# cloneofsimo/paint-with-words-sd

Hardware: AMD Instinct MI355X
Metric: 512x512 images/sec (30 steps, CFG) SD1.5+PwW (higher is better)
Workload: dtype bf16

## Files before the change

### paint-with-words-sd_amd/build.py

```python
import os
import subprocess
import sys

HERE = os.path.dirname(os.path.abspath(__file__))
REPO = os.path.dirname(HERE)
CSRC = os.path.join(HERE, "csrc")
LIB = os.path.join(HERE, "pww_hip", "libpww_hip.so")
LIB_EXPERIMENTS = os.path.join(HERE, "pww_hip", "libpww_hip_experiments.so")
UNITS = [("pww_api.hip", [], ""), ("pww_attn.hip", [], ""), ("pww_cross.hip", [], ""), ("pww_cross_lean.hip", [], ""), ("pww_reduce.hip", [], ""),
         ("pww_mask.hip", [], ""), ("pww_qproj.hip", [], ""), ("pww_norm.hip", [], ""), ("pww_blocks.hip", [], ""), ("pww_conv.hip", [], ""), ("pww_probs.hip", [], ""),
         ("pww_attn_inst.hip", ["-DPWW_INST_F16"], ".f16"), ("pww_attn_inst.hip", ["-DPWW_INST_BF16"], ".bf16"),
         ("pww_cross_inst.hip", ["-DPWW_INST_F16", "-DPWW_INST_NW=2"], ".f16.nw2"), ("pww_cross_inst.hip", ["-DPWW_INST_F16", "-DPWW_INST_NW=4"], ".f16.nw4"),
         ("pww_cross_inst.hip", ["-DPWW_INST_BF16", "-DPWW_INST_NW=2"], ".bf16.nw2"), ("pww_cross_inst.hip", ["-DPWW_INST_BF16", "-DPWW_INST_NW=4"], ".bf16.nw4")]
EXPERIMENT_UNITS = [("pww_cross_out.hip", [], "")]
_ATTN_HEADERS = ["pww_tile.h", "pww_attn_core.h", "pww_cross_tile.h"]
SIDE_FLAGS = ["-fvisibility=hidden"]
SIDE_LIBS = {
    "long": ("pww_long.hip", _ATTN_HEADERS, "the long-prompt launches"),
    "scope": ("pww_scope.hip", _ATTN_HEADERS, "cross-attention with per-head / per-row score statistics"),
    "linear": ("pww_linear.hip", [], "linear layers with a bias / residual / GEGLU epilogue"),
    "regions": ("pww_regions.hip", [], "region masks and the per-pixel blend of the noise predictions"),
    "lora": ("pww_lora.hip", [], "the per-row low-rank update of unmerged LoRA adapters"),
}
SIDE_LIBS_CONV = {
    "convtail": ("pww_conv_tail.hip", [], "conv2 of a ResnetBlock2D with the 1 x 1 shortcut as further K-slabs"),
}
SIDE_LIBS_EXTRA = {
    "canvas": ("pww_canvas.hip", [], "canvases larger than the UNet's window: the windows' gather and the combine of their noise predictions"),
}
ALL_SIDE_LIBS = {**SIDE_LIBS, **SIDE_LIBS_CONV, **SIDE_LIBS_EXTRA}
SOURCES = sorted({u[0] for u in UNITS + EXPERIMENT_UNITS})
HEADERS = ["pww_common.h", "pww_tile.h", "pww_attn_core.h", "pww_attn_kernel.h", "pww_cross_tile.h", "pww_cross_kernel.h", os.path.join(REPO, "include", "pww_hip.h")]
SIDE_PATHS = {n: os.path.join(HERE, "pww_hip", "libpww_hip_%s.so" % n) for n in ALL_SIDE_LIBS}
SIDE_UNITS = {n: [(v[0], SIDE_FLAGS, "")] for n, v in ALL_SIDE_LIBS.items()}
LIB_LONG, LIB_SCOPE, LIB_LINEAR, LIB_REGIONS, LIB_LORA = (SIDE_PATHS[n] for n in ("long", "scope", "linear", "regions", "lora"))
LONG_UNITS, SCOPE_UNITS, LINEAR_UNITS, REGIONS_UNITS, LORA_UNITS = (SIDE_UNITS[n] for n in ("long", "scope", "linear", "regions", "lora"))
LIB_CONVTAIL, CONVTAIL_UNITS = SIDE_PATHS["convtail"], SIDE_UNITS["convtail"]
LIB_CANVAS, CANVAS_UNITS = SIDE_PATHS["canvas"], SIDE_UNITS["canvas"]
SIDE_PUBLIC_HEADERS = {"canvas": ["pww_hip_regions.h"]}
HIPCC = os.environ.get("HIPCC", "/opt/rocm/bin/hipcc")
FLAGS = ["--offload-arch=gfx950", "-O3", "-std=c++17", "-fPIC", "-Wall",
         "-Wno-unused-function", "-mllvm", "-amdgpu-kernarg-preload-count=16"]


PER_FILE_FLAGS = {"pww_mask.hip": ["-ffp-contract=off"], "pww_regions.hip": ["-ffp-contract=off"], "pww_canvas.hip": ["-ffp-contract=off"]}


def _newer(target, deps):
    if not os.path.exists(target):
        return True
    t = os.path.getmtime(target)
    return any(os.path.getmtime(d) > t for d in deps)


def _deps():
    return ([os.path.join(CSRC, s) for s in SOURCES] + [h if os.path.isabs(h) else os.path.join(CSRC, h) for h in HEADERS] + [__file__])


def _build(lib, units, defines, objdir, verbose, jobs=None):
    os.makedirs(objdir, exist_ok=True)
    order = sorted(units, key=lambda u: {"pww_cross_inst.hip": 0, "pww_attn_inst.hip": 1, "pww_cross_lean.hip": 2}.get(u[0], 3))
    jobs = jobs or max(2, min(len(order), os.cpu_count() or 4, int(os.environ.get("MAX_JOBS", 16))))
    pending, running, objs = list(order), [], []
    while pending or running:
        while pending and len(running) < jobs:
            src, defs, suffix = pending.pop(0)
            o = os.path.join(objdir, src + suffix + ".o")
            objs.append(o)
            cmd = [HIPCC] + FLAGS + defines + defs + PER_FILE_FLAGS.get(src, []) + ["-c", os.path.join(CSRC, src), "-o", o]
            if verbose:
                print(" ".join(cmd))
            running.append((cmd, subprocess.Popen(cmd, stdout=subprocess.PIPE, stderr=subprocess.STDOUT, text=True)))
        cmd, p = running.pop(0)
        out, _ = p.communicate()
        if p.returncode != 0:
            for _, q in running:
                q.kill()
            raise RuntimeError("hipcc failed: %s\n%s" % (" ".join(cmd), out))
        if verbose and out.strip():
            print(out)
    subprocess.run([HIPCC, "--offload-arch=gfx950", "-shared", "-fPIC", "-s"] + sorted(objs) + ["-o", lib], check=True)
    return lib


def build_lib(force=False, verbose=False):
    if not force and not _newer(LIB, _deps()):
        return LIB
    return _build(LIB, UNITS, [], os.path.join(HERE, "build"), verbose)


def build_experiments(force=False, verbose=False):
    if not force and not _newer(LIB_EXPERIMENTS, _deps()):
        return LIB_EXPERIMENTS
    return _build(LIB_EXPERIMENTS, UNITS + EXPERIMENT_UNITS, ["-DPWW_EXPERIMENTS=1"], os.path.join(HERE, "build", "experiments"), verbose)


def build_side(name, force=False, verbose=False):
    unit, headers, _ = ALL_SIDE_LIBS[name]
    lib = SIDE_PATHS[name]
    public = ["pww_hip.h", "pww_hip_%s.h" % name] + SIDE_PUBLIC_HEADERS.get(name, [])
    deps = [os.path.join(CSRC, f) for f in [unit, "pww_common.h", "pww_side_host.h"] + headers] + [os.path.join(REPO, "include", h) for h in public] + [__file__]
    if not force and not _newer(lib, deps):
        return lib
    return _build(lib, SIDE_UNITS[name], [], os.path.join(HERE, "build", name), verbose)


def build_long(force=False, verbose=False): return build_side("long", force, verbose)
def build_scope(force=False, verbose=False): return build_side("scope", force, verbose)
def build_linear(force=False, verbose=False): return build_side("linear", force, verbose)
def build_regions(force=False, verbose=False): return build_side("regions", force, verbose)
def build_lora(force=False, verbose=False): return build_side("lora", force, verbose)
def build_convtail(force=False, verbose=False): return build_side("convtail", force, verbose)
def build_canvas(force=False, verbose=False): return build_side("canvas", force, verbose)


def _build_check(exe, lib, libname, defines, force):
    src = os.path.join(REPO, "tests", "native", "attn_check.cpp")
    if not force and not _newer(exe, [src, lib, os.path.join(REPO, "include", "pww_hip.h")]):
        return exe
    cmd = [HIPCC, "--offload-arch=gfx950", "-O2", "-std=c++17"] + defines + [src, "-o", exe, "-L" + os.path.dirname(lib), "-l" + libname,
                                                                              "-Wl,-rpath,$ORIGIN/../../paint-with-words-sd_amd/pww_hip"]
    subprocess.run(cmd, check=True)
    return exe


def build_native_check(force=False):
    return _build_check(os.path.join(REPO, "tests", "native", "attn_check"), build_lib(), "pww_hip", [], force)


def build_native_check_experiments(force=False):
    return _build_check(os.path.join(REPO, "tests", "native", "attn_check_experiments"), build_experiments(), "pww_hip_experiments", ["-DPWW_EXPERIMENTS=1"], force)


if __name__ == "__main__":
    force = "--force" in sys.argv
    print(build_lib(force=force, verbose=True))
    print(build_native_check(force=force))
    for name in ALL_SIDE_LIBS:
        print(build_side(name, force=force, verbose=True))
    if "--experiments" in sys.argv:
        print(build_experiments(force=force, verbose=True))
        print(build_native_check_experiments(force=force))
```

### paint-with-words-sd_amd/pww_hip/_lib.py

```python
import ctypes
import os

_HERE = os.path.dirname(os.path.abspath(__file__))
LIB_PATH = os.environ.get("PWW_HIP_LIB", os.path.join(_HERE, "libpww_hip.so"))
EXPERIMENTS_LIB_PATH = os.environ.get("PWW_HIP_EXPERIMENTS_LIB", os.path.join(_HERE, "libpww_hip_experiments.so"))

LONG_LIB_PATH = os.environ.get("PWW_HIP_LONG_LIB", os.path.join(_HERE, "libpww_hip_long.so"))
SCOPE_LIB_PATH = os.environ.get("PWW_HIP_SCOPE_LIB", os.path.join(_HERE, "libpww_hip_scope.so"))
LINEAR_LIB_PATH = os.environ.get("PWW_HIP_LINEAR_LIB", os.path.join(_HERE, "libpww_hip_linear.so"))
REGIONS_LIB_PATH = os.environ.get("PWW_HIP_REGIONS_LIB", os.path.join(_HERE, "libpww_hip_regions.so"))
LORA_LIB_PATH = os.environ.get("PWW_HIP_LORA_LIB", os.path.join(_HERE, "libpww_hip_lora.so"))
CONVTAIL_LIB_PATH = os.environ.get("PWW_HIP_CONVTAIL_LIB", os.path.join(_HERE, "libpww_hip_convtail.so"))
CANVAS_LIB_PATH = os.environ.get("PWW_HIP_CANVAS_LIB", os.path.join(_HERE, "libpww_hip_canvas.so"))

PWW_OK, PWW_EINVAL, PWW_ENOTSUP, PWW_EHIP = 0, -22, -95, -5
MIN_VERSION = 127
DTYPE_F16, DTYPE_BF16 = 0, 1
LAYOUT_NCHW, LAYOUT_NHWC = 0, 1
ACT_NONE, ACT_SILU = 0, 1
LINEAR_NONE, LINEAR_BIAS, LINEAR_BIAS_RESIDUAL, LINEAR_BIAS_GEGLU = 0, 1, 2, 3
MAX_HEAD_DIM = 160

EXPORTS = ("pww_version", "pww_has_experiments", "pww_last_error", "pww_device_arch", "pww_self_attn_fwd", "pww_cross_attn_fwd",
           "pww_cross_attn_fwd_stat", "pww_cross_attn_fwd_stat_ex",
           "pww_qk_reduce", "pww_mask_build", "pww_mask_build_rgb", "pww_mask_build_f32", "pww_resize_tokens", "pww_gauss_blur", "pww_inpaint_prep", "pww_cfg_combine", "pww_store_f32",
           "pww_workspace_bytes", "pww_profile_arm", "pww_profile_elapsed_us", "pww_profile_reset", "pww_debug_timeline", "pww_debug_path_counts",
           "pww_debug_last_attn_route",
           "pww_qproj_stat", "pww_qproj_parts", "pww_cross_attn_fwd_parts", "pww_mask_build_f32_levels", "pww_qk_parts", "pww_qk_parts_count",
           "pww_group_norm_fwd", "pww_group_norm_workspace_bytes", "pww_add_layer_norm", "pww_add_layer_norm_bias", "pww_geglu", "pww_bias_residual",
           "pww_conv3x3_workspace_bytes", "pww_conv3x3_fwd", "pww_cross_attn_probs")
EXPERIMENT_EXPORTS = ("pww_cross_attn_fwd_fused", "pww_cross_attn_fwd_fused_ex", "pww_cross_fused_workspace_bytes", "pww_cross_fused_state_bytes",
                      "pww_cross_attn_fwd_parts_out", "pww_cross_attn_out_supported")


LONG_EXPORTS = ("pww_long_version", "pww_long_last_error", "pww_long_qk_parts", "pww_long_qk_parts_count", "pww_long_cross_attn_fwd_parts",
                "pww_long_cross_attn_probs", "pww_long_profile_arm", "pww_long_profile_elapsed_us")
LONG_MIN_VERSION = 100
LONG_MIN_KEYS, LONG_MAX_KEYS = 129, 256


SCOPE_EXPORTS = ("pww_scope_version", "pww_scope_last_error", "pww_scope_head_parts_count", "pww_scope_head_parts", "pww_scope_cross_attn_fwd")
SCOPE_MIN_VERSION = 100
SCOPE_HEAD, SCOPE_ROW = 1, 2


LINEAR_EXPORTS = ("pww_linear_version", "pww_linear_last_error", "pww_linear_workspace_bytes", "pww_linear_fwd")
LINEAR_MIN_VERSION = 100


REGIONS_EXPORTS = ("pww_regions_version", "pww_regions_last_error", "pww_regions_masks", "pww_regions_combine")
REGIONS_MIN_VERSION = 100
REGIONS_MAX, REGIONS_MAX_PLANE, REGIONS_MAX_FEATHER = 8, 9216, 8.0


LORA_EXPORTS = ("pww_lora_version", "pww_lora_last_error", "pww_lora_fwd")
LORA_MIN_VERSION = 100
LORA_MAX_ADAPTERS, LORA_MAX_RANK, LORA_MAX_SEGMENTS = 8, 128, 3


CONVTAIL_EXPORTS = ("pww_convtail_version", "pww_convtail_last_error", "pww_convtail_workspace_bytes", "pww_convtail_fwd")
CONVTAIL_MIN_VERSION = 100


CANVAS_EXPORTS = ("pww_canvas_version", "pww_canvas_last_error", "pww_canvas_gather", "pww_canvas_combine")
CANVAS_MIN_VERSION = 100
CANVAS_MAX_WINDOWS, CANVAS_MAX_RAMP, CANVAS_MIN_WINDOW, CANVAS_MAX_WINDOW = 64, 64, 8, 128


class AttnDesc(ctypes.Structure):
    _fields_ = [("dtype", ctypes.c_int32), ("B", ctypes.c_int32), ("H", ctypes.c_int32), ("N", ctypes.c_int32),
                ("M", ctypes.c_int32), ("D", ctypes.c_int32),
                ("q_stride", ctypes.c_int64 * 3), ("k_stride", ctypes.c_int64 * 3),
                ("v_stride", ctypes.c_int64 * 3), ("o_stride", ctypes.c_int64 * 3),
                ("scale", ctypes.c_float), ("bias_stride", ctypes.c_int64 * 4)]


class CrossOpts(ctypes.Structure):
    _fields_ = [("size", ctypes.c_uint32), ("bias_cols", ctypes.c_int32), ("coeff_scalar_dev", ctypes.c_void_p),
                ("bias_compact", ctypes.c_void_p), ("col_idx", ctypes.c_void_p), ("R", ctypes.c_int32), ("gated_images", ctypes.c_int32),
                ("compact_stride", ctypes.c_int64 * 2), ("col_idx_stride", ctypes.c_int64)]


class QprojDesc(ctypes.Structure):
    _fields_ = [("dtype", ctypes.c_int32), ("B", ctypes.c_int32), ("N", ctypes.c_int32), ("Cin", ctypes.c_int32), ("H", ctypes.c_int32),
                ("D", ctypes.c_int32), ("M", ctypes.c_int32), ("x_stride", ctypes.c_int64 * 2), ("q_stride", ctypes.c_int64 * 2),
                ("k_stride", ctypes.c_int64 * 2)]


class GnDesc(ctypes.Structure):
    _fields_ = [("dtype", ctypes.c_int32), ("layout", ctypes.c_int32), ("B", ctypes.c_int32), ("C", ctypes.c_int32), ("HW", ctypes.c_int32),
                ("G", ctypes.c_int32), ("eps", ctypes.c_float), ("act", ctypes.c_int32), ("add_stride", ctypes.c_int32), ("_pad", ctypes.c_int32)]


class LnDesc(ctypes.Structure):
    _fields_ = [("dtype", ctypes.c_int32), ("C", ctypes.c_int32), ("rows", ctypes.c_int64), ("a_stride", ctypes.c_int64), ("x_stride", ctypes.c_int64),
                ("s_stride", ctypes.c_int64), ("y_stride", ctypes.c_int64), ("eps", ctypes.c_float), ("_pad", ctypes.c_int32)]


class ConvDesc(ctypes.Structure):
    _fields_ = [("size", ctypes.c_uint32), ("dtype", ctypes.c_int32), ("B", ctypes.c_int32), ("Hin", ctypes.c_int32), ("Win", ctypes.c_int32),
                ("Cin", ctypes.c_int32), ("Cout", ctypes.c_int32), ("stride", ctypes.c_int32), ("upsample", ctypes.c_int32), ("tile_n", ctypes.c_int32),
                ("splitk", ctypes.c_int32), ("_pad", ctypes.c_int32)]


class LinearDesc(ctypes.Structure):
    _fields_ = [("size", ctypes.c_uint32), ("dtype", ctypes.c_int32), ("M", ctypes.c_int32), ("N", ctypes.c_int32), ("K", ctypes.c_int32),
                ("epilogue", ctypes.c_int32), ("x_stride", ctypes.c_int64), ("y_stride", ctypes.c_int64), ("r_stride", ctypes.c_int64),
                ("tile_n", ctypes.c_int32), ("splitk", ctypes.c_int32)]


class ProbsDesc(ctypes.Structure):
    _fields_ = [("size", ctypes.c_uint32), ("images", ctypes.c_int32), ("accumulate", ctypes.c_int32), ("weight", ctypes.c_float),
                ("out_stride", ctypes.c_int64 * 2)]


class LoraDesc(ctypes.Structure):
    _fields_ = [("size", ctypes.c_uint32), ("dtype", ctypes.c_int32), ("R", ctypes.c_int32), ("T", ctypes.c_int32), ("K", ctypes.c_int32),
                ("N", ctypes.c_int32), ("n_seg", ctypes.c_int32), ("rank", ctypes.c_int32), ("n_adapters", ctypes.c_int32), ("_pad", ctypes.c_int32),
                ("x_row_stride", ctypes.c_int64), ("x_tok_stride", ctypes.c_int64), ("y_row_stride", ctypes.c_int64), ("y_tok_stride", ctypes.c_int64)]


class ConvTailDesc(ctypes.Structure):
    _fields_ = [("size", ctypes.c_uint32), ("dtype", ctypes.c_int32), ("B", ctypes.c_int32), ("H", ctypes.c_int32), ("W", ctypes.c_int32),
                ("Cin", ctypes.c_int32), ("C2", ctypes.c_int32), ("Cout", ctypes.c_int32), ("tile_n", ctypes.c_int32), ("splitk", ctypes.c_int32)]


class Region(ctypes.Structure):
    _fields_ = [("r", ctypes.c_uint8), ("g", ctypes.c_uint8), ("b", ctypes.c_uint8), ("_pad", ctypes.c_uint8),
                ("strength", ctypes.c_float)]


class PwwHipError(RuntimeError):
    pass


_lib = None
_exp = None


def _bind(lib, experiments):
    vp, i32, i64, f32 = ctypes.c_void_p, ctypes.c_int32, ctypes.c_int64, ctypes.c_float
    lib.pww_version.restype = ctypes.c_int
    if lib.pww_version() // 100 != 1 or lib.pww_version() < MIN_VERSION:
        raise PwwHipError("libpww_hip ABI version %d.%02d is not 1.x >= 1.%02d (rebuild: python paint-with-words-sd_amd/build.py)"
                          % (lib.pww_version() // 100, lib.pww_version() % 100, MIN_VERSION % 100))
    lib.pww_last_error.restype = ctypes.c_char_p
    lib.pww_device_arch.argtypes = [ctypes.c_char_p, ctypes.c_size_t]
    lib.pww_self_attn_fwd.argtypes = [vp, vp, vp, vp, ctypes.POINTER(AttnDesc), vp]
    lib.pww_cross_attn_fwd.argtypes = [vp, vp, vp, vp, vp, vp, ctypes.POINTER(AttnDesc), vp]
    lib.pww_cross_attn_fwd_stat.argtypes = [vp, vp, vp, vp, vp, vp, i32, ctypes.c_double, f32, vp, ctypes.POINTER(AttnDesc), vp]
    lib.pww_cross_attn_fwd_stat_ex.argtypes = [vp, vp, vp, vp, vp, vp, i32, ctypes.c_double, f32, vp, ctypes.POINTER(AttnDesc),
                                               ctypes.POINTER(CrossOpts), vp]
    lib.pww_qproj_stat.argtypes = [vp, vp, vp, vp, vp, ctypes.POINTER(QprojDesc), i32, vp, ctypes.c_size_t, vp]
    lib.pww_qproj_stat.restype = ctypes.c_int
    lib.pww_qproj_parts.argtypes = [ctypes.POINTER(QprojDesc)]
    lib.pww_qproj_parts.restype = ctypes.c_int32
    lib.pww_cross_attn_fwd_parts.argtypes = [vp, vp, vp, vp, vp, i32, f32, vp, ctypes.POINTER(AttnDesc), vp, i32, vp, ctypes.POINTER(CrossOpts), vp]
    lib.pww_cross_attn_fwd_parts.restype = ctypes.c_int
    lib.pww_qk_parts.argtypes = [vp, vp, vp, ctypes.POINTER(AttnDesc), i32, i32, vp, ctypes.c_size_t, vp]
    lib.pww_qk_parts.restype = ctypes.c_int
    lib.pww_qk_parts_count.argtypes = [ctypes.POINTER(AttnDesc)]
    lib.pww_qk_parts_count.restype = ctypes.c_int32
    lib.pww_mask_build_f32_levels.argtypes = [vp, i32, i32, i32, vp, vp, i32, vp, vp, vp, vp, vp]
    lib.pww_mask_build_f32_levels.restype = ctypes.c_int
    lib.pww_group_norm_workspace_bytes.argtypes = [ctypes.POINTER(GnDesc)]
    lib.pww_group_norm_workspace_bytes.restype = ctypes.c_size_t
    lib.pww_group_norm_fwd.argtypes = [vp, vp, vp, vp, vp, vp, ctypes.POINTER(GnDesc), vp, ctypes.c_size_t, vp]
    lib.pww_group_norm_fwd.restype = ctypes.c_int
    lib.pww_add_layer_norm.argtypes = [vp, vp, vp, vp, vp, vp, ctypes.POINTER(LnDesc), vp]
    lib.pww_add_layer_norm.restype = ctypes.c_int
    lib.pww_add_layer_norm_bias.argtypes = [vp, vp, vp, vp, vp, vp, vp, ctypes.POINTER(LnDesc), vp]
    lib.pww_add_layer_norm_bias.restype = ctypes.c_int
    lib.pww_geglu.argtypes = [vp, vp, ctypes.c_int64, i32, ctypes.c_int64, ctypes.c_int64, i32, vp]
    lib.pww_geglu.restype = ctypes.c_int
    lib.pww_bias_residual.argtypes = [vp, vp, vp, vp, i32, i32, i32, i32, i32, vp]
    lib.pww_bias_residual.restype = ctypes.c_int
    lib.pww_conv3x3_workspace_bytes.argtypes = [ctypes.POINTER(ConvDesc)]
    lib.pww_conv3x3_workspace_bytes.restype = ctypes.c_size_t
    lib.pww_conv3x3_fwd.argtypes = [vp, vp, vp, vp, vp, ctypes.POINTER(ConvDesc), vp, ctypes.c_size_t, vp]
    lib.pww_conv3x3_fwd.restype = ctypes.c_int
    lib.pww_cross_attn_probs.argtypes = [vp, vp, vp, vp, i32, ctypes.c_double, f32, vp, ctypes.POINTER(AttnDesc), ctypes.POINTER(CrossOpts), vp,
                                         ctypes.POINTER(ProbsDesc), vp]
    lib.pww_cross_attn_probs.restype = ctypes.c_int
    lib.pww_debug_timeline.argtypes = [vp, ctypes.c_size_t]
    lib.pww_debug_timeline.restype = None
    lib.pww_debug_path_counts.argtypes = [vp]
    lib.pww_debug_path_counts.restype = None
    lib.pww_debug_last_attn_route.argtypes = [ctypes.POINTER(i32), ctypes.c_int]
    lib.pww_debug_last_attn_route.restype = ctypes.c_int
    lib.pww_qk_reduce.argtypes = [vp, vp, ctypes.POINTER(AttnDesc), vp, vp, ctypes.c_size_t, vp]
    lib.pww_mask_build.argtypes = [vp, i32, i32, vp, i32, vp, vp, i32, vp, vp, vp, vp, vp]
    lib.pww_mask_build_rgb.argtypes = [vp, i32, i32, vp, i32, vp, vp, i32, i32, vp, vp]
    lib.pww_mask_build_f32.argtypes = [vp, i32, i32, i32, vp, vp, i32, i32, vp, vp]
    lib.pww_resize_tokens.argtypes = [vp, i32, i32, i32, i32, i32, i32, vp, vp]
    lib.pww_gauss_blur.argtypes = [vp, vp, i32, i32, vp, i32, vp, vp]
    lib.pww_inpaint_prep.argtypes = [vp, vp, i32, i32, i32, i32, vp, vp, vp, vp]
    lib.pww_cfg_combine.argtypes = [vp, vp, f32, vp, i64, i32, vp]
    lib.pww_store_f32.argtypes = [vp, ctypes.POINTER(ctypes.c_float), i32, vp]
    lib.pww_store_f32.restype = ctypes.c_int
    lib.pww_workspace_bytes.argtypes = [ctypes.POINTER(AttnDesc)]
    lib.pww_workspace_bytes.restype = ctypes.c_size_t
    lib.pww_profile_arm.argtypes = []
    lib.pww_profile_arm.restype = ctypes.c_int
    lib.pww_profile_elapsed_us.argtypes = [i32, ctypes.POINTER(ctypes.c_float)]
    lib.pww_profile_elapsed_us.restype = ctypes.c_int
    lib.pww_profile_reset.argtypes = []
    lib.pww_profile_reset.restype = None
    for name in ("pww_device_arch", "pww_self_attn_fwd", "pww_cross_attn_fwd", "pww_cross_attn_fwd_stat", "pww_cross_attn_fwd_stat_ex", "pww_qk_reduce",
                 "pww_mask_build", "pww_mask_build_rgb", "pww_mask_build_f32", "pww_resize_tokens", "pww_gauss_blur", "pww_inpaint_prep", "pww_cfg_combine"):
        getattr(lib, name).restype = ctypes.c_int
    lib.pww_has_experiments.restype = ctypes.c_int
    if experiments:
        lib.pww_cross_attn_fwd_fused.argtypes = [vp, vp, vp, vp, vp, i32, f32, vp, ctypes.POINTER(AttnDesc), vp, vp, ctypes.c_size_t, vp, ctypes.c_size_t, vp]
        lib.pww_cross_attn_fwd_fused_ex.argtypes = [vp, vp, vp, vp, vp, i32, f32, vp, ctypes.POINTER(AttnDesc), vp, vp, ctypes.c_size_t, vp,
                                                    ctypes.c_size_t, ctypes.POINTER(CrossOpts), vp]
        lib.pww_cross_attn_fwd_fused.restype = lib.pww_cross_attn_fwd_fused_ex.restype = ctypes.c_int
        lib.pww_cross_fused_workspace_bytes.argtypes = [ctypes.POINTER(AttnDesc)]
        lib.pww_cross_fused_workspace_bytes.restype = ctypes.c_size_t
        lib.pww_cross_fused_state_bytes.argtypes = [ctypes.POINTER(AttnDesc)]
        lib.pww_cross_fused_state_bytes.restype = ctypes.c_size_t
        lib.pww_cross_attn_fwd_parts_out.argtypes = [vp, vp, vp, vp, vp, i32, f32, vp, ctypes.POINTER(AttnDesc), vp, i32, vp, ctypes.POINTER(CrossOpts),
                                                     vp, vp, vp, ctypes.POINTER(ctypes.c_int64), vp]
        lib.pww_cross_attn_fwd_parts_out.restype = ctypes.c_int
        lib.pww_cross_attn_out_supported.argtypes = [ctypes.POINTER(AttnDesc), ctypes.c_int32, ctypes.c_int32]
        lib.pww_cross_attn_out_supported.restype = ctypes.c_int32
    return lib


def load():
    global _lib
    if _lib is not None:
        return _lib
    if not os.path.isfile(LIB_PATH):
        raise PwwHipError(
            "libpww_hip.so not found at %s. Build it with `python paint-with-words-sd_amd/build.py` "
            "(or __graft_entry__.build()). There is no CPU/PyTorch fallback for the PwW kernels." % LIB_PATH)
    lib = ctypes.CDLL(LIB_PATH)
    _lib = _bind(lib, hasattr(lib, "pww_has_experiments") and bool(lib.pww_has_experiments()))
    return _lib


def has_experiments():
    return bool(load().pww_has_experiments())


def load_experiments():
    global _exp
    if _exp is not None:
        return _exp
    if has_experiments():
        _exp = load()
        return _exp
    if not os.path.isfile(EXPERIMENTS_LIB_PATH):
        raise PwwHipError("libpww_hip_experiments.so not found at %s: this entry point is not part of the product library. Build it with "
                          "`python paint-with-words-sd_amd/build.py --experiments` (tests: the `experiments_lib` fixture does)." % EXPERIMENTS_LIB_PATH)
    lib = ctypes.CDLL(EXPERIMENTS_LIB_PATH)
    lib.pww_has_experiments.restype = ctypes.c_int
    if not lib.pww_has_experiments():
        raise PwwHipError("%s was not built with -DPWW_EXPERIMENTS=1" % EXPERIMENTS_LIB_PATH)
    _exp = _bind(lib, True)
    return _exp


_P = ctypes.POINTER
_vp, _i32, _i64, _f32, _f64, _sz, _int = ctypes.c_void_p, ctypes.c_int32, ctypes.c_int64, ctypes.c_float, ctypes.c_double, ctypes.c_size_t, ctypes.c_int
_HINT = "(rebuild: python paint-with-words-sd_amd/build.py, or __graft_entry__.build())"
SIDE = {
    "long": dict(path="LONG_LIB_PATH", exports=LONG_EXPORTS, min_version=LONG_MIN_VERSION, missing_ok=False, needs="prompts longer than 77 tokens need it", sigs={
        "pww_long_qk_parts": ([_vp, _vp, _vp, _P(AttnDesc), _i32, _i32, _vp, _sz, _vp], _int),
        "pww_long_qk_parts_count": ([_P(AttnDesc)], _i32),
        "pww_long_cross_attn_fwd_parts": ([_vp, _vp, _vp, _vp, _vp, _i32, _f32, _vp, _P(AttnDesc), _vp, _i32, _vp, _P(CrossOpts), _vp], _int),
        "pww_long_cross_attn_probs": ([_vp, _vp, _vp, _vp, _i32, _f64, _f32, _vp, _P(AttnDesc), _P(CrossOpts), _vp, _P(ProbsDesc), _vp], _int),
        "pww_long_profile_arm": ([], _int),
        "pww_long_profile_elapsed_us": ([_P(_f32)], _int)}),
    "scope": dict(path="SCOPE_LIB_PATH", exports=SCOPE_EXPORTS, min_version=SCOPE_MIN_VERSION, missing_ok=True, needs="per-head / per-row score statistics need it", sigs={
        "pww_scope_head_parts_count": ([_P(AttnDesc)], _i32),
        "pww_scope_head_parts": ([_vp, _vp, _vp, _P(AttnDesc), _i32, _vp, _sz, _vp], _int),
        "pww_scope_cross_attn_fwd": ([_vp, _vp, _vp, _vp, _vp, _i32, _i32, _f32, _vp, _P(AttnDesc), _vp, _i32, _vp, _P(CrossOpts), _vp], _int)}),
    "linear": dict(path="LINEAR_LIB_PATH", exports=LINEAR_EXPORTS, min_version=LINEAR_MIN_VERSION, missing_ok=False, needs="linear layers on the native kernel need it", sigs={
        "pww_linear_workspace_bytes": ([_P(LinearDesc)], _sz),
        "pww_linear_fwd": ([_vp, _vp, _vp, _vp, _vp, _P(LinearDesc), _vp, _sz, _vp], _int)}),
    "regions": dict(path="REGIONS_LIB_PATH", exports=REGIONS_EXPORTS, min_version=REGIONS_MIN_VERSION, missing_ok=False, needs="region prompts need it", sigs={
        "pww_regions_masks": ([_vp, _i32, _i32, _vp, _i32, _f32, _vp, _vp], _int),
        "pww_regions_combine": ([_vp, _vp, _vp, _vp, _f32, _vp, _i32, _i32, _i32, _i64, _i32, _vp], _int)}),
}
SIDE_MORE = {
    "lora": dict(path="LORA_LIB_PATH", exports=LORA_EXPORTS, min_version=LORA_MIN_VERSION, missing_ok=False, needs="LoRA adapters on the native kernel need it", sigs={
        "pww_lora_fwd": ([_vp, _vp, _vp, _vp, _vp, _vp, _P(LoraDesc), _vp], _int)}),
}
SIDE_CONV = {
    "convtail": dict(path="CONVTAIL_LIB_PATH", exports=CONVTAIL_EXPORTS, min_version=CONVTAIL_MIN_VERSION, missing_ok=True, needs="conv2 with the shortcut as K-slabs needs it", sigs={
        "pww_convtail_workspace_bytes": ([_P(ConvTailDesc)], _sz),
        "pww_convtail_fwd": ([_vp, _vp, _vp, _vp, _vp, _vp, _vp, _P(ConvTailDesc), _vp, _sz, _vp], _int)}),
}
SIDE_EXTRA = {
    "canvas": dict(path="CANVAS_LIB_PATH", exports=CANVAS_EXPORTS, min_version=CANVAS_MIN_VERSION, missing_ok=False, needs="canvases larger than the window need it", sigs={
        "pww_canvas_gather": ([_vp, _vp, _P(_i32), _i32, _P(_i32), _i32, _i32, _i32, _i32, _i32, _i32, _f32, _i32, _i32, _vp], _int),
        "pww_canvas_combine": ([_vp, _vp, _vp, _vp, _f32, _vp, _P(_i32), _i32, _P(_i32), _i32, _i32, _i32, _i32, _i32, _i32, _i32, _i32, _i32, _vp], _int)}),
}
_side = {}


def side_spec(name):
    for table in (SIDE, SIDE_MORE, SIDE_CONV):
        if name in table:
            return table[name]
    return SIDE_EXTRA[name]


def load_side(name):
    lib = _side.get(name)
    if lib is not None:
        return lib
    spec = side_spec(name)
    path, so, pre = globals()[spec["path"]], "libpww_hip_%s.so" % name, "pww_%s_" % name
    if not os.path.isfile(path):
        if spec["missing_ok"]:
            return None
        raise PwwHipError("%s not found at %s: %s %s" % (so, path, spec["needs"], _HINT))
    try:
        lib = ctypes.CDLL(path)
        getattr(lib, pre + "version").restype = _int
        version = getattr(lib, pre + "version")()
    except (OSError, AttributeError) as e:
        raise PwwHipError("%s at %s cannot be loaded: %s %s" % (so, path, e, _HINT))
    if version // 100 != 1 or version < spec["min_version"]:
        raise PwwHipError("%s ABI version %d is not 1.x >= %d %s" % (so[:-3], version, spec["min_version"], _HINT))
    missing = [n for n in spec["exports"] if not hasattr(lib, n)]
    if missing:
        raise PwwHipError("%s at %s lacks %s %s" % (so, path, missing, _HINT))
    for fn, (argtypes, restype) in spec["sigs"].items():
        getattr(lib, fn).argtypes, getattr(lib, fn).restype = argtypes, restype
    getattr(lib, pre + "last_error").restype = ctypes.c_char_p
    lib.pww_last_error = getattr(lib, pre + "last_error")
    _side[name] = lib
    return lib


def load_long():
    lib = _side.get("long")
    return lib if lib is not None else load_side("long")


def load_scope():
    lib = _side.get("scope")
    return lib if lib is not None else load_side("scope")


def load_linear():
    lib = _side.get("linear")
    return lib if lib is not None else load_side("linear")


def load_regions():
    lib = _side.get("regions")
    return lib if lib is not None else load_side("regions")


def load_lora():
    lib = _side.get("lora")
    return lib if lib is not None else load_side("lora")


def load_convtail():
    lib = _side.get("convtail")
    return lib if lib is not None else load_side("convtail")


def load_canvas():
    lib = _side.get("canvas")
    return lib if lib is not None else load_side("canvas")


class experiments:

    def __enter__(self):
        global _lib
        load()
        self._prev = _lib
        _lib = load_experiments()
        return _lib

    def __exit__(self, *exc):
        global _lib
        _lib = self._prev
        return False


def check(rc, what, lib=None):
    if rc != PWW_OK:
        msg = (lib or load()).pww_last_error().decode("utf-8", "replace")
        raise PwwHipError("%s failed (rc=%d): %s" % (what, rc, msg))


def device_arch():
    buf = ctypes.create_string_buffer(64)
    check(load().pww_device_arch(buf, 64), "pww_device_arch")
    return buf.value.decode()
```

### paint-with-words-sd_amd/pww_hip/blocks.py

```python
import os
import types
import warnings

import torch
import torch.nn as nn
import torch.nn.functional as F

from . import ops

FUSED_NORM = os.environ.get("PWW_FUSED_NORM", "1") != "0"
BATCHED_TEMB = os.environ.get("PWW_BATCHED_TEMB", "1") != "0"
FOLD_CONV_BIAS = os.environ.get("PWW_FOLD_CONV_BIAS", "1") != "0"
CONV1X1_AS_LINEAR = os.environ.get("PWW_CONV1X1_AS_LINEAR", "1") != "0"
LINEAR = os.environ.get("PWW_LINEAR", "1")
CONV3X3 = os.environ.get("PWW_CONV3X3", "1") != "0"
CONV_SHORTCUT = os.environ.get("PWW_CONV_SHORTCUT", "1") != "0"


_STATS = {k: [0, 0] for k in ("group_norm", "resnet_block", "transformer_block", "geglu", "conv1x1", "conv3x3", "linear", "conv_shortcut")}
_UNRATED = ("conv1x1", "conv3x3", "linear", "conv_shortcut")
_warned = set()


def stats():
    out = {k: {"fused": v[0], "declined": v[1]} for k, v in _STATS.items()}
    rated = [v for k, v in _STATS.items() if k not in _UNRATED]
    tot = sum(v[0] + v[1] for v in rated)
    out["hit_rate"] = (sum(v[0] for v in rated) / tot) if tot else None
    return out


def reset_stats():
    for v in _STATS.values():
        v[0] = v[1] = 0


def _count(op, fused, x=None, reason=None):
    _STATS[op][0 if fused else 1] += 1
    if not fused and FUSED_NORM and torch.is_tensor(x) and x.is_cuda and x.dtype in (torch.float16, torch.bfloat16):
        key = (op, reason)
        if key not in _warned:
            _warned.add(key)
            warnings.warn("pww_hip.blocks: %s call on a HIP %s tensor handed to the stock op (%s); pww_hip.blocks.stats() counts them"
                          % (op, str(x.dtype).split(".")[-1], reason or "shape / dtype the kernels do not take"), stacklevel=3)


def _why_not(x):
    if torch.is_autocast_enabled():
        return "torch.autocast is on: the norms run in fp32 there"
    if torch.is_grad_enabled() and torch.is_tensor(x) and x.requires_grad:
        return "autograd is recording: the kernels are forward-only"
    return None


def _takes(x, norm):
    if not (FUSED_NORM and torch.is_tensor(x) and x.is_cuda and x.dim() == 4 and x.dtype in (torch.float16, torch.bfloat16)):
        return False
    B, C, H, W = x.shape
    w = norm.weight
    return (C % 8 == 0 and (H * W) % 8 == 0 and C % norm.num_groups == 0 and norm.num_groups <= 32 and C <= 4096
            and (w is None or w.dtype == x.dtype) and not torch.is_autocast_enabled()
            and not (torch.is_grad_enabled() and (x.requires_grad or (w is not None and w.requires_grad))))


def fused_group_norm(norm, x, add=None, act=None):
    if _takes(x, norm) and (add is None or add.dtype == x.dtype):
        return ops.group_norm(x, norm.num_groups, norm.weight, norm.bias, norm.eps, add=add, act=act)
    if add is not None:
        x = x + add[:, :, None, None]
    y = F.group_norm(x, norm.num_groups, norm.weight, norm.bias, norm.eps)
    return F.silu(y) if act == "silu" else y


def _group_norm_forward(self, x, *args, **kwargs):
    if args or kwargs or not _takes(x, self):
        _count("group_norm", False, x, "unexpected arguments" if (args or kwargs) else _why_not(x))
        return self._pww_orig_forward(x, *args, **kwargs)
    _count("group_norm", True)
    return fused_group_norm(self, x)


def _is_silu(m):
    return m is None or isinstance(m, nn.SiLU) or m is F.silu


def _resnet_covered(m):
    return (isinstance(getattr(m, "norm1", None), nn.GroupNorm) and isinstance(getattr(m, "norm2", None), nn.GroupNorm)
            and hasattr(m, "conv1") and hasattr(m, "conv2") and getattr(m, "upsample", None) is None and getattr(m, "downsample", None) is None
            and getattr(m, "time_embedding_norm", "default") == "default" and _is_silu(getattr(m, "nonlinearity", None)))


class TembProjections:

    def __init__(self):
        self.linears = []
        self.width = 0
        self._sig = None
        self._w = self._b = None

    def register(self, block):
        lin = block.time_emb_proj
        slot = (self, self.width, lin.out_features)
        self.linears.append((lin, self.width, lin.out_features))
        self.width += (lin.out_features + 7) // 8 * 8
        return slot

    def _signature(self, dtype, device):
        sig = [dtype, device]
        for lin, _, _ in self.linears:
            sig.append((lin.weight.data_ptr(), lin.weight._version, lin.weight.dtype))
            sig.append(None if lin.bias is None else (lin.bias.data_ptr(), lin.bias._version))
        return tuple(sig)

    def project(self, temb):
        hit = temb.__dict__.get("_pww_temb_proj")
        if hit is not None and hit[0] is self and hit[2] == (temb._version, temb.data_ptr()):
            return hit[1]
        sig = self._signature(temb.dtype, temb.device)
        if sig != self._sig:
            w = torch.zeros(self.width, self.linears[0][0].in_features, dtype=temb.dtype, device=temb.device)
            b = torch.zeros(self.width, dtype=temb.dtype, device=temb.device)
            for lin, off, n in self.linears:
                w[off:off + n] = lin.weight.detach().to(temb.dtype)
                if lin.bias is not None:
                    b[off:off + n] = lin.bias.detach().to(temb.dtype)
            self._w, self._b, self._sig = w, b, sig
        out = F.linear(F.silu(temb), self._w, self._b)
        temb.__dict__["_pww_temb_proj"] = (self, out, (temb._version, temb.data_ptr()))
        return out


def _conv_no_bias(conv, x):
    return F.conv2d(x, conv.weight, None, conv.stride, conv.padding, conv.dilation, conv.groups)


def _plain_conv(conv):
    return isinstance(conv, nn.Conv2d) and conv.bias is not None and conv.padding_mode == "zeros" and type(conv).forward is nn.Conv2d.forward \
        and "forward" not in conv.__dict__ and not conv._forward_hooks and not conv._forward_pre_hooks


def _resnet_forward(self, *args, **kwargs):
    covered = 1 <= len(args) <= 2 and set(kwargs) <= {"temb"} and not (len(args) == 2 and kwargs)
    input_tensor = args[0] if args else None
    if not covered or not _takes(input_tensor, self.norm1):
        _count("resnet_block", False, input_tensor, ("a call beyond (input_tensor, temb): %d positional, keywords %s" % (len(args), sorted(kwargs))) if not covered else _why_not(input_tensor))
        return self._pww_orig_forward(*args, **kwargs)
    temb = args[1] if len(args) == 2 else kwargs.get("temb")
    _count("resnet_block", True)
    fold = FOLD_CONV_BIAS and _plain_conv(self.conv1) and _plain_conv(self.conv2) and self.conv1.bias.dtype == input_tensor.dtype
    h = fused_group_norm(self.norm1, input_tensor, act="silu")
    if fold and _conv3x3_route(self.conv1, h):
        h = ops.conv3x3(h, self.conv1.weight)
    else:
        h = _conv_no_bias(self.conv1, h) if fold else self.conv1(h)
    add = None
    if temb is not None and getattr(self, "time_emb_proj", None) is not None:
        slot = self.__dict__.get("_pww_temb_slot")
        if slot is not None and temb.dtype == h.dtype and temb.dim() == 2 and not torch.is_grad_enabled():
            add = slot[0].project(temb)[:, slot[1]:slot[1] + slot[2]]
        else:
            add = self.time_emb_proj(F.silu(temb))
        if add.dtype != h.dtype:
            add = add.to(h.dtype)
    if fold and _takes(h, self.norm2):
        h = ops.group_norm(h, self.norm2.num_groups, self.norm2.weight, self.norm2.bias, self.norm2.eps, add=add, act="silu", pre_bias=self.conv1.bias)
    else:
        if fold:
            h = h + self.conv1.bias[None, :, None, None]
        h = fused_group_norm(self.norm2, h, add=add, act="silu")
    dropout = getattr(self, "dropout", None)
    if dropout is not None:
        h = dropout(h)
    scale = getattr(self, "output_scale_factor", 1.0)
    shortcut = getattr(self, "conv_shortcut", None)
    if shortcut is not None:
        if _conv_shortcut_route(self, shortcut, h, input_tensor, fold, scale):
            return ops.conv3x3_shortcut(h, self.conv2.weight, self.conv2.bias, input_tensor, shortcut.weight, shortcut.bias)
        input_tensor = shortcut(input_tensor)
    if fold and input_tensor.dtype == h.dtype and input_tensor.shape == (h.shape[0], self.conv2.out_channels) + h.shape[2:] and _conv3x3_route(self.conv2, h):
        out = ops.conv3x3(h, self.conv2.weight, self.conv2.bias, residual=input_tensor)
    elif fold and input_tensor.dtype == h.dtype and input_tensor.shape[1] % 8 == 0:
        out = ops.bias_residual(input_tensor, _conv_no_bias(self.conv2, h), self.conv2.bias)
    else:
        out = input_tensor + self.conv2(h)
    return out if scale == 1.0 else out / scale


def _is_conv3x3(m):
    return (isinstance(m, nn.Conv2d) and type(m).forward is nn.Conv2d.forward and m.kernel_size == (3, 3) and m.stride in ((1, 1), (2, 2))
            and m.padding == (1, 1) and m.dilation == (1, 1) and m.groups == 1 and m.padding_mode == "zeros")


STOCK_FROM_ROWS = 16384


def _conv3x3_route(conv, x, upsample=False):
    ok = (CONV3X3 and FUSED_NORM and torch.is_tensor(x) and x.dim() == 4 and _is_conv3x3(conv) and not torch.is_autocast_enabled() and not (torch.is_grad_enabled() and (x.requires_grad or conv.weight.requires_grad))
          and (conv.bias is None or conv.bias.dtype == x.dtype) and ops.conv3x3_takes(x, conv.weight, conv.stride[0], upsample)
          and (upsample or x.shape[0] * ((x.shape[2] - 1) // conv.stride[0] + 1) * ((x.shape[3] - 1) // conv.stride[0] + 1) < STOCK_FROM_ROWS))
    _STATS["conv3x3"][0 if ok else 1] += 1
    return ok


def _conv_shortcut_route(block, shortcut, h, x, fold, scale):
    own = shortcut.__dict__.get("forward")
    ok = (CONV_SHORTCUT and fold and scale == 1.0 and _is_conv1x1(shortcut) and shortcut.bias is not None
          and (own is None or getattr(own, "__func__", None) is _conv1x1_forward) and not shortcut._forward_hooks and not shortcut._forward_pre_hooks
          and torch.is_tensor(x) and x.dim() == 4 and x.dtype == h.dtype == shortcut.weight.dtype == shortcut.bias.dtype
          and x.is_contiguous(memory_format=torch.channels_last)
          and not (torch.is_grad_enabled() and (x.requires_grad or shortcut.weight.requires_grad))
          and _is_conv3x3(block.conv2) and block.conv2.stride == (1, 1) and ops.conv3x3_shortcut_takes(h, block.conv2.weight, x, shortcut.weight)
          and ops._lib.load_convtail() is not None)
    if ok:
        ok = _conv3x3_route(block.conv2, h)
        if not ok:
            _STATS["conv3x3"][1] -= 1
    _STATS["conv_shortcut"][0 if ok else 1] += 1
    return ok


def _conv3x3_forward(self, x, *args, **kwargs):
    if not args and not kwargs and _conv3x3_route(self, x):
        return ops.conv3x3(x, self.weight, self.bias, stride=self.stride[0])
    return self._pww_orig_forward(x, *args, **kwargs)


def _upsample_conv(m):
    if getattr(m, "use_conv_transpose", False) or not getattr(m, "use_conv", True):
        return None
    conv = getattr(m, "Conv2d_0", None) if getattr(m, "name", "conv") != "conv" else getattr(m, "conv", None)
    return conv if _is_conv3x3(conv) and conv.stride == (1, 1) and "forward" not in conv.__dict__ and not conv._forward_hooks and not conv._forward_pre_hooks else None


def _upsample_forward(self, *args, **kwargs):
    plain = 1 <= len(args) <= 2 and set(kwargs) <= {"output_size"} and all(a is None for a in list(args[1:]) + list(kwargs.values()))
    x = args[0] if plain and not (len(args) == 2 and kwargs) else None
    conv = _upsample_conv(self)
    if x is not None and conv is not None and x.dim() == 4 and (getattr(self, "channels", None) in (None, x.shape[1])) and _conv3x3_route(conv, x, upsample=True):
        return ops.conv3x3(x, conv.weight, conv.bias, upsample=True)
    return self._pww_orig_forward(*args, **kwargs)


def _conv1x1_forward(self, x, *args, **kwargs):
    if (not args and not kwargs and FUSED_NORM and CONV1X1_AS_LINEAR and torch.is_tensor(x) and x.is_cuda and x.dim() == 4 and x.dtype == self.weight.dtype
            and x.shape[2] * x.shape[3] > 1 and x.is_contiguous(memory_format=torch.channels_last) and not torch.is_autocast_enabled()):
        B, C, H, W = x.shape
        _STATS["conv1x1"][0] += 1
        y = F.linear(x.permute(0, 2, 3, 1).reshape(B * H * W, C), self.weight.reshape(self.out_channels, C), self.bias)
        return y.view(B, H, W, self.out_channels).permute(0, 3, 1, 2)
    _STATS["conv1x1"][1] += 1
    return self._pww_orig_forward(x, *args, **kwargs)


def _is_conv1x1(m):
    return (isinstance(m, nn.Conv2d) and type(m).forward is nn.Conv2d.forward and m.kernel_size == (1, 1) and m.stride == (1, 1) and m.padding == (0, 0)
            and m.dilation == (1, 1) and m.groups == 1 and m.padding_mode == "zeros")


def _ln_takes(x, norm):
    return (FUSED_NORM and torch.is_tensor(x) and x.is_cuda and x.dtype in (torch.float16, torch.bfloat16) and x.dim() >= 2
            and len(norm.normalized_shape) == 1 and x.shape[-1] == norm.normalized_shape[0] and x.shape[-1] % 8 == 0 and x.shape[-1] <= 2048
            and (norm.weight is None or norm.weight.dtype == x.dtype) and not torch.is_autocast_enabled()
            and not (torch.is_grad_enabled() and (x.requires_grad or (norm.weight is not None and norm.weight.requires_grad))))


def _transformer_block_covered(m):
    return (all(isinstance(getattr(m, n, None), nn.LayerNorm) for n in ("norm1", "norm2", "norm3")) and hasattr(m, "attn1") and hasattr(m, "attn2")
            and hasattr(m, "ff") and not getattr(m, "only_cross_attention", False))


def _transformer_block_forward(self, *args, **kwargs):
    covered = 1 <= len(args) <= 2 and set(kwargs) <= {"context", "timestep"} and kwargs.get("timestep") is None and not (len(args) == 2 and "context" in kwargs)
    hidden_states = args[0] if args else None
    if not covered or not _ln_takes(hidden_states, self.norm1):
        _count("transformer_block", False, hidden_states, ("a call beyond (hidden_states, context, timestep=None): %d positional, keywords %s" % (len(args), sorted(kwargs)))
               if not covered else _why_not(hidden_states))
        return self._pww_orig_forward(*args, **kwargs)
    context = args[1] if len(args) == 2 else kwargs.get("context")
    _count("transformer_block", True)
    h = hidden_states
    n = ops.add_layer_norm(h, self.norm1.weight, self.norm1.bias, self.norm1.eps)
    h, n = ops.add_layer_norm(h, self.norm2.weight, self.norm2.bias, self.norm2.eps, a=self.attn1(n))
    h, n = ops.add_layer_norm(h, self.norm3.weight, self.norm3.bias, self.norm3.eps, a=self.attn2(n, context=context))
    lin = _ff_output_linear(self.ff) if LINEAR != "0" else None
    if lin is not None:
        g = self.ff.net[0](n)
        if _linear_route(g, lin.weight, lin.bias, "residual", residual=h):
            return ops.linear(g, lin.weight, lin.bias, residual=h)
        return lin(g) + h
    return self.ff(n) + h


def _ff_output_linear(ff):
    net = getattr(ff, "net", None)
    if net is None or len(net) != 3 or type(ff).__name__ != "FeedForward" or "forward" in ff.__dict__:
        return None
    owner = next((c for c in type(ff).__mro__ if "forward" in c.__dict__), None)
    if owner is None or owner.__name__ != "FeedForward":
        return None
    act, drop, lin = net[0], net[1], net[2]
    if act.__class__.__name__ != "GEGLU" or not isinstance(drop, nn.Dropout) or (drop.training and drop.p > 0):
        return None
    if type(lin) is not nn.Linear or lin.bias is None or lin._forward_hooks or lin._forward_pre_hooks or "forward" in lin.__dict__ or ff._forward_hooks or ff._forward_pre_hooks:
        return None
    return lin


LINEAR_ROUTES = frozenset([
    (8192, 320, 2560, "geglu"),
    (2048, 640, 5120, "geglu"),
    (512, 1280, 10240, "geglu"),
    (128, 1280, 10240, "geglu"),
    (512, 5120, 1280, "residual"),
])


def _linear_route(x, weight, bias, epilogue, residual=None):
    ok = (LINEAR != "0" and FUSED_NORM and not torch.is_autocast_enabled() and torch.is_tensor(x) and bias is not None and bias.dtype == x.dtype
          and not (torch.is_grad_enabled() and (x.requires_grad or weight.requires_grad)) and ops.linear_takes(x, weight, epilogue == "geglu", bias=bias, residual=residual)
          and (LINEAR == "force" or (x.numel() // x.shape[-1], x.shape[-1], weight.shape[0], epilogue) in LINEAR_ROUTES))
    _STATS["linear"][0 if ok else 1] += 1
    return ok


def _plain_linear(lin):
    return type(lin) is nn.Linear and lin.bias is not None and not lin._forward_hooks and not lin._forward_pre_hooks and "forward" not in lin.__dict__


def _geglu_forward(self, x, *args, **kwargs):
    if args or kwargs:
        _count("geglu", False, x, "arguments beyond (hidden_states): %s" % (sorted(kwargs) or len(args)))
        return self._pww_orig_forward(x, *args, **kwargs)
    if _plain_linear(self.proj) and _linear_route(x, self.proj.weight, self.proj.bias, "geglu"):
        _count("geglu", True)
        return ops.linear(x, self.proj.weight, self.proj.bias, geglu=True)
    h = self.proj(x)
    if FUSED_NORM and h.is_cuda and h.dtype in (torch.float16, torch.bfloat16) and h.shape[-1] % 16 == 0 and not torch.is_autocast_enabled() \
            and not (torch.is_grad_enabled() and h.requires_grad):
        _count("geglu", True)
        return ops.geglu(h)
    _count("geglu", False, h, _why_not(h))
    a, gate = h.chunk(2, dim=-1)
    return a * F.gelu(gate)


def install_blocks(unet):
    n_res = n_gn = 0
    owned = set()
    plans = {}
    for m in unet.modules():
        if m.__class__.__name__ == "ResnetBlock2D" and _resnet_covered(m):
            if "_pww_orig_forward" not in m.__dict__:
                m.__dict__["_pww_orig_forward"] = m.forward
                m.forward = types.MethodType(_resnet_forward, m)
                lin = getattr(m, "time_emb_proj", None)
                if BATCHED_TEMB and isinstance(lin, nn.Linear):
                    m.__dict__["_pww_temb_slot"] = plans.setdefault(lin.in_features, TembProjections()).register(m)
            owned.update((id(m.norm1), id(m.norm2), id(m.conv1), id(m.conv2)))
            n_res += 1
    for m in unet.modules():
        name, fwd = m.__class__.__name__, None
        if isinstance(m, nn.GroupNorm) and id(m) not in owned:
            fwd = _group_norm_forward
            n_gn += 1
        elif name == "BasicTransformerBlock" and _transformer_block_covered(m):
            fwd = _transformer_block_forward
        elif name == "GEGLU" and isinstance(getattr(m, "proj", None), nn.Linear):
            fwd = _geglu_forward
        elif _is_conv1x1(m):
            fwd = _conv1x1_forward
        elif name == "Upsample2D" and _upsample_conv(m) is not None:
            fwd = _upsample_forward
            owned.add(id(_upsample_conv(m)))
        elif _is_conv3x3(m) and id(m) not in owned:
            fwd = _conv3x3_forward
        if fwd is not None and "_pww_orig_forward" not in m.__dict__:
            m.__dict__["_pww_orig_forward"] = m.forward
            m.forward = types.MethodType(fwd, m)
    return n_res, n_gn


def uninstall_blocks(unet):
    for m in unet.modules():
        if "_pww_orig_forward" in m.__dict__:
            del m.__dict__["_pww_orig_forward"]
            m.__dict__.pop("forward", None)
            m.__dict__.pop("_pww_temb_slot", None)
```

### paint-with-words-sd_amd/pww_hip/ops.py

```python
import ctypes

import torch

from . import _lib
from ._lib import AttnDesc, CrossOpts, ProbsDesc, QprojDesc, Region, PwwHipError

_DT = {torch.float16: _lib.DTYPE_F16, torch.bfloat16: _lib.DTYPE_BF16}


def _stream():
    return ctypes.c_void_p(torch.cuda.current_stream().cuda_stream)


def _ptr(t):
    return ctypes.c_void_p(t.data_ptr()) if t is not None else ctypes.c_void_p(0)


def _require_gpu(*tensors):
    for t in tensors:
        if t is not None and not t.is_cuda:
            raise PwwHipError("pww_hip ops need tensors on a HIP device (got %s); there is no CPU path" % t.device)


def _rows_ok(t):
    return t.stride(-1) == 1 and t.stride(0) % 8 == 0 and t.stride(1) % 8 == 0 and t.data_ptr() % 16 == 0


def _desc(q, k, v, o, heads, scale):
    if q.dim() != 3 or k.dim() != 3 or (v is not None and v.dim() != 3):
        raise PwwHipError("q/k/v must be [batch, tokens, heads*dim] tensors")
    B, N, C = q.shape
    M = k.shape[1]
    if C % heads:
        raise PwwHipError("channels %d not divisible by heads %d" % (C, heads))
    if k.shape[2] != C or k.shape[0] not in (1, B):
        raise PwwHipError("key shape %s does not match query shape %s" % (tuple(k.shape), tuple(q.shape)))
    if v is not None and tuple(v.shape) != tuple(k.shape):
        raise PwwHipError("value shape %s differs from key shape %s" % (tuple(v.shape), tuple(k.shape)))
    if M < 1 or N < 1 or B < 1:
        raise PwwHipError("empty attention problem (B=%d N=%d M=%d)" % (B, N, M))
    D = C // heads
    d = AttnDesc()
    d.dtype = _DT[q.dtype]
    d.B, d.H, d.N, d.M, d.D = B, heads, N, M, D
    d.q_stride[:] = [q.stride(0), D, q.stride(1)]
    kb = k.stride(0) if k.shape[0] == B and B > 1 else 0
    d.k_stride[:] = [kb, D, k.stride(1)]
    if v is not None:
        d.v_stride[:] = [v.stride(0) if v.shape[0] == B and B > 1 else 0, D, v.stride(1)]
    if o is not None:
        d.o_stride[:] = [o.stride(0), D, o.stride(1)]
    d.scale = float(scale)
    return d


def _prep(t):
    if t.dtype not in _DT:
        raise PwwHipError("dtype %s unsupported (float16 / bfloat16)" % t.dtype)
    return t if _rows_ok(t) else t.contiguous()


STAT_NONE, STAT_MAX, STAT_MIN, STAT_MEAN, STAT_STD, STAT_ABSMAX, STAT_ALL = 0, 1, 2, 3, 4, 5, 6
FUSED_MAX_KEYS = 128
MAX_HEAD_DIM = _lib.MAX_HEAD_DIM
LONG_MAX_KEYS = _lib.LONG_MAX_KEYS
COMPACT_MAX_R = 32


class FusedScratch:

    def __init__(self):
        self.state = None
        self.ws = None
        self._err_index = 0
        self._retired = []
        self._err_sites = {}

    def _alloc(self, current, nbytes, device, zero):
        if current is not None and current.device == device and current.numel() * 8 >= nbytes:
            return current
        if torch.cuda.is_current_stream_capturing():
            raise PwwHipError("fused cross-attention buffers must exist before hipGraph capture (run one eager call first)")
        if current is not None:
            self._retired.append(current)
        n = (nbytes + 7) // 8
        return (torch.zeros if zero else torch.empty)((n,), dtype=torch.int64, device=device)

    def ensure(self, lib, d, device):
        lib = _lib.load_experiments()
        self.state = self._alloc(self.state, int(lib.pww_cross_fused_state_bytes(ctypes.byref(d))), device, True)
        self.ws = self._alloc(self.ws, int(lib.pww_cross_fused_workspace_bytes(ctypes.byref(d))), device, False)
        self._err_index = d.B * d.H + d.B
        self._err_sites.setdefault(id(self.state), (self.state, set()))[1].add(self._err_index)
        return self.state, self.ws

    def error_word(self):
        return None if self.state is None else self.state.view(torch.int32)[self._err_index]

    def error_words(self):
        return [buf.view(torch.int32)[i] for buf, idxs in self._err_sites.values() for i in sorted(idxs)]

    def error(self):
        words = self.error_words()
        return bool(words) and bool(torch.stack(words).ne(0).any().item())

    def reset(self):
        for t in [self.state] + self._retired:
            if t is not None:
                t.zero_()


class FusedErrorWatch:

    def __init__(self):
        self.pending = []

    def post(self, modules):
        scratches = [m.__dict__["_pww_fused_scratch"] for m in modules if "_pww_fused_scratch" in getattr(m, "__dict__", {})]
        words = [w for s in scratches for w in s.error_words()]
        if not words:
            return False
        flag = torch.stack(words).ne(0).any().to(torch.int32)
        host = torch.empty((), dtype=torch.int32).pin_memory()
        host.copy_(flag, non_blocking=True)
        ev = torch.cuda.Event()
        ev.record()
        self.pending.append((ev, host, scratches))
        return True

    def poll(self, wait=False):
        while self.pending:
            ev, host, scratches = self.pending[0]
            if wait:
                ev.synchronize()
            elif not ev.query():
                return
            self.pending.pop(0)
            if int(host.item()) != 0:
                torch.cuda.synchronize()
                for s in scratches:
                    s.reset()
                self.pending.clear()
                raise PwwHipError(_TIMEOUT_MESSAGE)


_TIMEOUT_MESSAGE = ("a fused cross-attention launch timed out waiting for its own workgroups (the GPU is shared with another process or "
                    "stream?); its outputs are NaN and were discarded. State re-zeroed. Set PWW_FUSED_CROSS=0 to use the two-launch "
                    "path on a shared device.")


def check_fused_errors(modules):
    scratches = [m.__dict__["_pww_fused_scratch"] for m in modules if "_pww_fused_scratch" in getattr(m, "__dict__", {})]
    words = [w for s in scratches for w in s.error_words()]
    if not words:
        return
    if bool(torch.stack(words).ne(0).any().item()):
        torch.cuda.synchronize()
        for s in scratches:
            s.reset()
        raise PwwHipError(_TIMEOUT_MESSAGE)


def _cross_opts(B, N, coeff_dev, bias_cols, compact, gated=0):
    if coeff_dev is None and not bias_cols and compact is None and not gated:
        return None
    op = CrossOpts()
    op.size = ctypes.sizeof(CrossOpts)
    op.bias_cols = int(bias_cols or 0)
    op.gated_images = int(gated or 0)
    if coeff_dev is not None:
        if coeff_dev.dtype != torch.float32 or coeff_dev.numel() != 1 or not coeff_dev.is_cuda:
            raise PwwHipError("coeff_dev must be a one-element float32 device tensor")
        op.coeff_scalar_dev = coeff_dev.data_ptr()
    if compact is not None:
        wc, idx = compact
        if wc.dtype != torch.float32 or idx.dtype != torch.int32 or wc.stride(-1) != 1 or idx.stride(-1) != 1:
            raise PwwHipError("compact bias: float32 values and int32 column indices, innermost stride 1")
        if wc.dim() == 2:
            wc = wc.unsqueeze(0)
        if idx.dim() == 1:
            idx = idx.unsqueeze(0)
        R = wc.shape[-1]
        if wc.shape[1] != N or wc.shape[0] not in (1, B) or idx.shape[-1] != R or idx.shape[0] not in (1, B):
            raise PwwHipError("compact bias shapes %s / %s do not fit B=%d N=%d" % (tuple(wc.shape), tuple(idx.shape), B, N))
        op.bias_compact, op.col_idx, op.R = wc.data_ptr(), idx.data_ptr(), R
        op.compact_stride[:] = [wc.stride(0) if wc.shape[0] == B and B > 1 else 0, wc.stride(1)]
        op.col_idx_stride = idx.stride(0) if idx.shape[0] == B and B > 1 else 0
        op.keep = (wc, idx)
    return op


def _opt_ref(op):
    return ctypes.byref(op) if op is not None else None


def _bias_view(bias, d):
    if bias.dtype != torch.float32:
        bias = bias.float()
    if bias.dim() == 3 and bias.shape[0] == d.B * d.H and d.B * d.H != 1:
        bias = bias.reshape(d.B, d.H, bias.shape[1], bias.shape[2])
    bias = torch.broadcast_to(bias, (d.B, d.H, d.N, d.M))
    d.bias_stride[:] = list(bias.stride())
    return bias


def _per_image_f32(t, B, name, expand=False):
    if t is None:
        return None
    t = t.to(torch.float32).reshape(-1).contiguous()
    if expand and t.numel() == 1 and B > 1:
        t = t.expand(B).contiguous()
    if t.numel() != B:
        raise PwwHipError("%s must have B=%d elements" % (name, B))
    return t


def _check_f64(t, name, *shape):
    if t is not None and (t.dtype != torch.float64 or t.dim() != len(shape) or not t.is_contiguous()
                          or any(not isinstance(s, str) and s != n for s, n in zip(shape, t.shape))):
        raise PwwHipError("%s must be a contiguous float64 [%s] tensor" % (name, ", ".join(["B"] + [str(s) for s in shape[1:]])))


def _attention_route(has_bias, stat, scratch, parts, M):
    if not has_bias:
        return "self"
    if stat is None:
        return "plain"
    if stat[0] is not None:
        return "stat"
    if stat[1] == STAT_NONE and parts is None and M > FUSED_MAX_KEYS:
        return "stat"
    return "parts" if scratch is None else "fused"


def attention_route(has_bias, stat, scratch, parts, M):
    route = _attention_route(has_bias, stat, scratch, parts, M)
    if route in ("parts", "stat") and stat[0] is None and scratch is None and long_keys(M):
        return "long"
    return route


def _launch_stat(lib, io, bias, coeff, d, stat, coeff_dev):
    stats, kind, scalar = stat
    _check_f64(stats, "stat: stats", d.B, 4)
    op = _cross_opts(d.B, d.N, coeff_dev, 0, None)
    _lib.check(lib.pww_cross_attn_fwd_stat_ex(*io, _ptr(bias), _ptr(stats), int(kind), float(d.H * d.N * d.M), float(scalar), _ptr(coeff),
                                              ctypes.byref(d), _opt_ref(op), _stream()), "pww_cross_attn_fwd_stat_ex")


def _parts_stat(d, stat, parts, missing):
    _, kind, scalar = stat
    if kind != STAT_NONE and parts is None:
        raise PwwHipError(missing)
    _check_f64(parts, "parts", d.B, "nparts", 4)
    return kind, scalar


def _parts_args(io, bias, coeff, d, kind, scalar, parts, stats_out, op):
    return (*io, _ptr(bias), int(kind), float(scalar), _ptr(coeff), ctypes.byref(d), _ptr(parts), int(parts.shape[1]) if parts is not None else 0,
            _ptr(stats_out), _opt_ref(op), _stream())


def _launch_parts(lib, io, bias, coeff, d, stat, parts, stats_out, coeff_dev, bias_cols, compact, gated):
    kind, scalar = _parts_stat(d, stat, parts, "a statistic formed outside the attention launch needs its partials (qproj_stat / qk_parts), or a "
                                               "FusedScratch for the in-launch form")
    if d.M > FUSED_MAX_KEYS:
        raise PwwHipError("the pass-2-only cross-attention launch takes at most %d keys (partials over more keys: fold them with "
                          "fold_parts and pass stat=(stats, kind, scalar))" % FUSED_MAX_KEYS)
    _check_f64(stats_out, "stats_out", d.B, 4)
    if compact is not None and (compact[0].shape[-1] > COMPACT_MAX_R or not _lib.has_experiments()):
        compact = None
    op = _cross_opts(d.B, d.N, coeff_dev, bias_cols, compact, gated)
    _lib.check(lib.pww_cross_attn_fwd_parts(*_parts_args(io, bias, coeff, d, kind, scalar, parts, stats_out, op)), "pww_cross_attn_fwd_parts")


def long_keys(M):
    return FUSED_MAX_KEYS < M <= LONG_MAX_KEYS


def _launch_long(io, bias, coeff, d, stat, parts, stats_out, coeff_dev, bias_cols, gated):
    kind, scalar = _parts_stat(d, stat, parts, "a statistic over %d keys needs its partials (long_qk_parts)" % d.M)
    _check_f64(stats_out, "stats_out", d.B, 4)
    op = _cross_opts(d.B, d.N, coeff_dev, bias_cols, None, gated)
    lib = _lib.load_long()
    want = int(lib.pww_long_qk_parts_count(ctypes.byref(d))) if parts is not None else 0
    if parts is not None and parts.shape[1] != want:
        raise PwwHipError("cross-attention over %d keys folds the partials of long_qk_parts (%d per image for this problem), got %d: the pass-2-only "
                          "launch of libpww_hip.so takes at most %d keys" % (d.M, want, parts.shape[1], FUSED_MAX_KEYS))
    _lib.check(lib.pww_long_cross_attn_fwd_parts(*_parts_args(io, bias, coeff, d, kind, scalar, parts, stats_out, op)),
               "pww_long_cross_attn_fwd_parts", lib)


def _launch_fused(io, bias, coeff, d, stat, scratch, device, stats_out, coeff_dev, bias_cols, compact, gated):
    _, kind, scalar = stat
    if d.M > FUSED_MAX_KEYS:
        raise PwwHipError("fused statistic needs a FusedScratch and at most %d keys" % FUSED_MAX_KEYS)
    xlib = _lib.load_experiments()
    state, ws = scratch.ensure(xlib, d, device)
    _check_f64(stats_out, "stats_out", d.B, 4)
    if compact is not None and compact[0].shape[-1] > COMPACT_MAX_R:
        compact = None
    op = _cross_opts(d.B, d.N, coeff_dev, bias_cols, compact, gated)
    _lib.check(xlib.pww_cross_attn_fwd_fused_ex(*io, _ptr(bias), int(kind), float(scalar), _ptr(coeff), ctypes.byref(d), _ptr(stats_out), _ptr(state),
                                                state.numel() * 8, _ptr(ws), ws.numel() * 8, _opt_ref(op), _stream()), "pww_cross_attn_fwd_fused_ex", xlib)


def attention(q, k, v, heads, scale, bias=None, bias_coeff=None, stat=None, scratch=None, stats_out=None, coeff_dev=None,
              bias_cols=0, compact=None, gated=0, parts=None):
    _require_gpu(q, k, v, bias, bias_coeff)
    if not (q.dtype == k.dtype == v.dtype):
        raise PwwHipError("q/k/v dtypes differ: %s %s %s" % (q.dtype, k.dtype, v.dtype))
    q, k, v = _prep(q), _prep(k), _prep(v)
    B, N, C = q.shape
    out = torch.empty((B, N, C), dtype=q.dtype, device=q.device)
    d = _desc(q, k, v, out, heads, scale)
    lib = _lib.load()
    route = attention_route(bias is not None, stat, scratch, parts, d.M)
    io = (_ptr(q), _ptr(k), _ptr(v), _ptr(out))
    if route != "self":
        bias = _bias_view(bias, d)
        bias_coeff = _per_image_f32(bias_coeff, B, "bias_coeff", expand=True)
    with torch.cuda.device(q.device):
        if route == "self":
            _lib.check(lib.pww_self_attn_fwd(*io, ctypes.byref(d), _stream()), "pww_self_attn_fwd")
        elif route == "plain":
            _lib.check(lib.pww_cross_attn_fwd(*io, _ptr(bias), _ptr(bias_coeff), ctypes.byref(d), _stream()), "pww_cross_attn_fwd")
        elif route == "stat":
            _launch_stat(lib, io, bias, bias_coeff, d, stat, coeff_dev)
        elif route == "parts":
            _launch_parts(lib, io, bias, bias_coeff, d, stat, parts, stats_out, coeff_dev, bias_cols, compact, gated)
        elif route == "long":
            _launch_long(io, bias, bias_coeff, d, stat, parts, stats_out, coeff_dev, bias_cols, gated)
        else:
            _launch_fused(io, bias, bias_coeff, d, stat, scratch, q.device, stats_out, coeff_dev, bias_cols, compact, gated)
    return out


def probs_buffer(images, N, M, device, zero=True):
    make = torch.zeros if zero else torch.empty
    return make((images, N, (M + 3) & ~3), dtype=torch.float32, device=device)[:, :, :M]


def attention_probs(q, k, heads, scale, bias=None, bias_coeff=None, stat=None, coeff_dev=None, images=0, out=None, accumulate=False, weight=1.0):
    _require_gpu(q, k, bias, bias_coeff, out)
    if q.dtype != k.dtype:
        raise PwwHipError("q/k dtypes differ: %s %s" % (q.dtype, k.dtype))
    q, k = _prep(q), _prep(k)
    d = _desc(q, k, None, None, heads, scale)
    B, N, M = d.B, d.N, d.M
    if M > LONG_MAX_KEYS:
        raise PwwHipError("attention_probs takes at most %d keys (got %d)" % (LONG_MAX_KEYS, M))
    n_img = int(images or 0)
    if n_img < 0 or n_img > B:
        raise PwwHipError("attention_probs: images = %d outside 0 .. B = %d" % (n_img, B))
    rows = n_img or B
    if bias is not None:
        bias = _bias_view(bias, d)
        bias_coeff = _per_image_f32(bias_coeff, B, "bias_coeff", expand=True)
    else:
        bias_coeff = None
    stats, kind, scalar = stat if stat is not None else (None, STAT_NONE, 1.0)
    _check_f64(stats, "stat: stats", B, 4)
    if stats is None and kind != STAT_NONE:
        raise PwwHipError("attention_probs: a statistic needs its [B, 4] statistics (qk_stats, or the stats_out of the attention launch)")
    if out is None:
        if accumulate:
            raise PwwHipError("attention_probs: accumulate needs `out`")
        out = probs_buffer(rows, N, M, q.device, zero=False)
    elif (out.dtype != torch.float32 or out.dim() != 3 or out.shape[0] < rows or out.shape[1] != N or out.shape[2] < M or out.stride(2) != 1
          or out.stride(1) % 4 or out.stride(0) % 4 or out.data_ptr() % 16 or out.device != q.device):
        raise PwwHipError("attention_probs: `out` must be an fp32 [>= %d, %d, >= %d] tensor on %s, 16-byte aligned, unit key stride, row / image strides "
                          "multiples of 4" % (rows, N, M, q.device))
    pd = ProbsDesc(ctypes.sizeof(ProbsDesc), n_img, int(bool(accumulate)), float(weight))
    pd.out_stride[:] = [out.stride(0), out.stride(1)]
    op = _cross_opts(B, N, coeff_dev, 0, None)
    lib = _lib.load_long() if long_keys(M) else _lib.load()
    launch, name = (lib.pww_long_cross_attn_probs, "pww_long_cross_attn_probs") if long_keys(M) else (lib.pww_cross_attn_probs, "pww_cross_attn_probs")
    with torch.cuda.device(q.device):
        _lib.check(launch(_ptr(q), _ptr(k), _ptr(bias), _ptr(stats), int(kind), float(d.H * N * M), float(scalar), _ptr(bias_coeff),
                          ctypes.byref(d), _opt_ref(op), _ptr(out), ctypes.byref(pd), _stream()), name, lib)
    return out


def attention_out_supported(q, k, heads, bias, weight, bias_cols=0):
    if q.dtype not in _DT or q.dim() != 3 or k.dim() != 3 or bias is None or not torch.is_tensor(weight):
        return False
    B, N, C = q.shape
    M = k.shape[1]
    if tuple(weight.shape) != (C, C) or weight.dtype != q.dtype or not weight.is_contiguous() or C % heads:
        return False
    d = AttnDesc()
    d.dtype = _DT[q.dtype]
    d.B, d.H, d.N, d.M, d.D = B, heads, N, M, C // heads
    d.q_stride[:] = [q.stride(0), C // heads, q.stride(1)]
    try:
        _bias_view(bias, d)
    except RuntimeError:
        return False
    return bool(_lib.load_experiments().pww_cross_attn_out_supported(ctypes.byref(d), C, int(bias_cols)))


def attention_out(q, k, v, heads, scale, bias, weight, weight_bias=None, residual=None, bias_coeff=None, stat=None, parts=None, stats_out=None,
                  coeff_dev=None, bias_cols=0, gated=0):
    _require_gpu(q, k, v, bias, bias_coeff, weight, weight_bias, residual)
    if not (q.dtype == k.dtype == v.dtype == weight.dtype):
        raise PwwHipError("q/k/v/weight dtypes differ: %s %s %s %s" % (q.dtype, k.dtype, v.dtype, weight.dtype))
    q, k, v = _prep(q), _prep(k), _prep(v)
    B, N, C = q.shape
    if tuple(weight.shape) != (C, C) or not weight.is_contiguous():
        raise PwwHipError("attention_out: weight must be a contiguous [%d, %d] tensor" % (C, C))
    if weight_bias is not None and (weight_bias.dtype != q.dtype or tuple(weight_bias.shape) != (C,) or not weight_bias.is_contiguous()):
        raise PwwHipError("attention_out: weight_bias must be a contiguous [%d] tensor of q's dtype" % C)
    if residual is not None and (residual.dtype != q.dtype or tuple(residual.shape) != (B, N, C) or residual.stride(2) != 1):
        raise PwwHipError("attention_out: residual must be a [B, N, C] tensor of q's dtype with unit channel stride")
    out = torch.empty((B, N, C), dtype=q.dtype, device=q.device)
    d = _desc(q, k, v, out, heads, scale)
    bias = _bias_view(bias, d)
    bias_coeff = _per_image_f32(bias_coeff, B, "bias_coeff", expand=True)
    if stat is not None and stat[0] is not None:
        raise PwwHipError("attention_out folds partials (stat = (None, kind, scalar), parts = qproj_stat / qk_parts output)")
    kind, scalar = _parts_stat(d, stat or (None, STAT_NONE, 1.0), parts, "attention_out: a statistic needs its partials (qproj_stat / qk_parts)")
    _check_f64(stats_out, "stats_out", B, 4)
    op = _cross_opts(B, N, coeff_dev, bias_cols, None, gated)
    rs = (ctypes.c_int64 * 2)(residual.stride(0), residual.stride(1)) if residual is not None else None
    lib = _lib.load_experiments()
    with torch.cuda.device(q.device):
        rc = lib.pww_cross_attn_fwd_parts_out(_ptr(q), _ptr(k), _ptr(v), _ptr(out), _ptr(bias), int(kind), float(scalar), _ptr(bias_coeff), ctypes.byref(d),
                                              _ptr(parts), int(parts.shape[1]) if parts is not None else 0, _ptr(stats_out),
                                              _opt_ref(op), _ptr(weight), _ptr(weight_bias), _ptr(residual), rs, _stream())
    _lib.check(rc, "pww_cross_attn_fwd_parts_out", lib)
    return out


def _qproj_desc(x, weight, k, heads):
    if x.dim() != 3 or k.dim() != 3 or weight.dim() != 2:
        raise PwwHipError("qproj: x [B, N, Cin], weight [C, Cin], k [B or 1, M, C]")
    B, N, Cin = x.shape
    C = weight.shape[0]
    if weight.shape[1] != Cin or k.shape[2] != C or k.shape[0] not in (1, B) or C % heads:
        raise PwwHipError("qproj: shapes do not fit (x %s, weight %s, k %s, heads %d)" % (tuple(x.shape), tuple(weight.shape), tuple(k.shape), heads))
    d = QprojDesc()
    d.dtype = _DT[x.dtype]
    d.B, d.N, d.Cin, d.H, d.D, d.M = B, N, Cin, heads, C // heads, k.shape[1]
    d.x_stride[:] = [x.stride(0), x.stride(1)]
    d.k_stride[:] = [k.stride(0) if k.shape[0] == B and B > 1 else 0, k.stride(1)]
    return d


def qproj_parts(x, weight, k, heads):
    if x.dtype not in _DT or not (x.dtype == weight.dtype == k.dtype) or k.shape[1] > FUSED_MAX_KEYS:
        return 0
    d = _qproj_desc(x, weight, k, heads)
    d.q_stride[:] = [x.shape[1] * weight.shape[0], weight.shape[0]]
    return int(_lib.load().pww_qproj_parts(ctypes.byref(d)))


def qproj_stat(x, weight, k, heads, kind, gate=None):
    _require_gpu(x, weight, k, gate)
    if not (x.dtype == weight.dtype == k.dtype):
        raise PwwHipError("qproj: dtypes differ: %s %s %s" % (x.dtype, weight.dtype, k.dtype))
    x, k = _prep(x), _prep(k)
    weight = weight if weight.is_contiguous() else weight.contiguous()
    B, N, Cin = x.shape
    C = weight.shape[0]
    q = torch.empty((B, N, C), dtype=x.dtype, device=x.device)
    d = _qproj_desc(x, weight, k, heads)
    d.q_stride[:] = [q.stride(0), q.stride(1)]
    lib = _lib.load()
    nparts = int(lib.pww_qproj_parts(ctypes.byref(d)))
    if nparts <= 0:
        raise PwwHipError("qproj_stat: unsupported shape (C = %d, head dim %d, Cin = %d): ask qproj_parts() first" % (C, C // heads, Cin))
    parts = torch.empty((B, nparts, 4), dtype=torch.float64, device=x.device)
    gate = _per_image_f32(gate, B, "gate")
    with torch.cuda.device(x.device):
        _lib.check(lib.pww_qproj_stat(_ptr(x), _ptr(weight), _ptr(q), _ptr(k), _ptr(gate), ctypes.byref(d), int(kind), _ptr(parts),
                                      parts.numel() * 8, _stream()), "pww_qproj_stat")
    return q, parts


def _stat_parts(name, load, q, k, heads, kind, gate, gated=0, per_head=False):
    _require_gpu(q, k, gate)
    if q.dtype != k.dtype:
        raise PwwHipError("%s: dtypes differ: %s %s" % (name, q.dtype, k.dtype))
    q, k = _prep(q), _prep(k)
    d = _desc(q, k, None, None, heads, 1.0)
    lib = load()
    nparts = int(getattr(lib, "pww_%s_count" % name)(ctypes.byref(d)))
    if nparts <= 0:
        raise PwwHipError("%s: unsupported problem %s x %s, %d heads" % (name, tuple(q.shape), tuple(k.shape), heads))
    B = q.shape[0]
    parts = torch.empty((B, heads, nparts, 4) if per_head else (B, nparts, 4), dtype=torch.float64, device=q.device)
    gate = _per_image_f32(gate, B, "gate")
    hint = () if per_head else (int(gated or 0),)
    with torch.cuda.device(q.device):
        _lib.check(getattr(lib, "pww_" + name)(_ptr(q), _ptr(k), _ptr(gate), ctypes.byref(d), int(kind), *hint, _ptr(parts), parts.numel() * 8, _stream()),
                   "pww_" + name, lib)
    return parts


def qk_parts(q, k, heads, kind, gate=None, gated=0):
    return _stat_parts("qk_parts", _lib.load, q, k, heads, kind, gate, gated)


def long_qk_parts(q, k, heads, kind, gate=None, gated=0):
    return _stat_parts("long_qk_parts", _lib.load_long, q, k, heads, kind, gate, gated)


SCOPE_HEAD, SCOPE_ROW = _lib.SCOPE_HEAD, _lib.SCOPE_ROW
_SCOPED_KINDS = (STAT_MAX, STAT_MIN, STAT_MEAN, STAT_STD, STAT_ABSMAX)


def scoped_available():
    return _lib.load_scope() is not None


def _scope_lib():
    lib = _lib.load_scope()
    if lib is None:
        raise PwwHipError("libpww_hip_scope.so not found at %s: per-head / per-row score statistics need it. Build it with "
                          "`python paint-with-words-sd_amd/build.py` (or __graft_entry__.build())." % _lib.SCOPE_LIB_PATH)
    return lib


def scope_head_parts(q, k, heads, kind, gate=None):
    return _stat_parts("scope_head_parts", _scope_lib, q, k, heads, kind, gate, per_head=True)


def attention_scoped(q, k, v, heads, scale, bias, kind, scope, scalar, gate=None, parts=None, stats_out=None, coeff_dev=None):
    _require_gpu(q, k, v, bias, gate, parts, stats_out)
    if not (q.dtype == k.dtype == v.dtype):
        raise PwwHipError("q/k/v dtypes differ: %s %s %s" % (q.dtype, k.dtype, v.dtype))
    if bias is None:
        raise PwwHipError("attention_scoped needs a bias map")
    if scope not in (SCOPE_HEAD, SCOPE_ROW) or kind not in _SCOPED_KINDS:
        raise PwwHipError("attention_scoped: scope %r / statistic %r outside SCOPE_HEAD, SCOPE_ROW / STAT_MAX ... STAT_ABSMAX" % (scope, kind))
    q, k, v = _prep(q), _prep(k), _prep(v)
    B, N, C = q.shape
    out = torch.empty((B, N, C), dtype=q.dtype, device=q.device)
    d = _desc(q, k, v, out, heads, scale)
    if d.M > FUSED_MAX_KEYS:
        raise PwwHipError("attention_scoped takes at most %d keys (got %d)" % (FUSED_MAX_KEYS, d.M))
    bias = _bias_view(bias, d)
    gate = _per_image_f32(gate, B, "gate", expand=True)
    if scope == SCOPE_HEAD:
        if parts is None:
            raise PwwHipError("attention_scoped: head scope folds the partials of scope_head_parts")
        _check_f64(parts, "parts", B, heads, "nparts", 4)
        _check_f64(stats_out, "stats_out", B, heads, 4)
    elif parts is not None or stats_out is not None:
        raise PwwHipError("attention_scoped: row scope takes no partials and writes no stats_out")
    op = _cross_opts(B, N, coeff_dev, 0, None)
    lib = _scope_lib()
    with torch.cuda.device(q.device):
        _lib.check(lib.pww_scope_cross_attn_fwd(_ptr(q), _ptr(k), _ptr(v), _ptr(out), _ptr(bias), int(kind), int(scope), float(scalar), _ptr(gate),
                                                ctypes.byref(d), _ptr(parts), int(parts.shape[2]) if parts is not None else 0, _ptr(stats_out),
                                                _opt_ref(op), _stream()), "pww_scope_cross_attn_fwd", lib)
    return out


def fold_parts(parts):
    return torch.stack([parts[:, :, 0].amax(1), parts[:, :, 1].amin(1), parts[:, :, 2].sum(1), parts[:, :, 3].sum(1)], dim=1)


def qk_stats(q, k, heads):
    _require_gpu(q, k)
    q, k = _prep(q), _prep(k)
    stats = torch.empty((q.shape[0], 4), dtype=torch.float64, device=q.device)
    d = _desc(q, k, None, None, heads, 1.0)
    lib = _lib.load()
    nbytes = int(lib.pww_workspace_bytes(ctypes.byref(d)))
    ws = torch.empty(((nbytes + 7) // 8,), dtype=torch.float64, device=q.device)
    with torch.cuda.device(q.device):
        _lib.check(lib.pww_qk_reduce(_ptr(q), _ptr(k), ctypes.byref(d), _ptr(stats), _ptr(ws), ws.numel() * 8, _stream()),
                   "pww_qk_reduce")
    return stats


def _regions_tensor(regions, device):
    arr = (Region * len(regions))()
    for i, (r, g, b, s) in enumerate(regions):
        arr[i] = Region(int(r), int(g), int(b), 0, float(s))
    raw = torch.frombuffer(bytearray(bytes(arr)), dtype=torch.uint8)
    return raw.to(device)


def _csr(cols, device):
    ptr, reg = [0], []
    for lst in cols:
        reg.extend(int(x) for x in lst)
        ptr.append(len(reg))
    col_ptr = torch.tensor(ptr, dtype=torch.int32).to(device)
    col_reg = torch.tensor(reg if reg else [0], dtype=torch.int32).to(device)
    return col_ptr, col_reg


def round_half_up_div(a, ratio):
    return (2 * a + ratio) // (2 * ratio)


def _level_rows(H, W, ratios):
    rows = {}
    for r in ratios:
        rows[r] = round_half_up_div(H, r) * round_half_up_div(W, r) if r > 0 else 0
        if rows[r] <= 0:
            raise PwwHipError("mask_build: image %dx%d too small for ratio %d" % (H, W, r))
    return rows


def mask_build(rgb, regions, cols, ratios=(8, 16, 32, 64)):
    _require_gpu(rgb)
    if rgb.dtype != torch.uint8 or rgb.dim() != 3 or rgb.shape[2] != 3:
        raise PwwHipError("rgb must be uint8 [H, W, 3]")
    rgb = rgb.contiguous()
    H, W = rgb.shape[:2]
    T = len(cols)
    dev = rgb.device
    rows = _level_rows(H, W, ratios)
    regs = _regions_tensor(regions, dev)
    col_ptr, col_reg = _csr(cols, dev)
    outs = {r: torch.empty((rows[r], T), dtype=torch.float32, device=dev) for r in ratios}
    lib = _lib.load()
    with torch.cuda.device(dev):
        if tuple(ratios) == (8, 16, 32, 64):
            rc = lib.pww_mask_build(_ptr(rgb), H, W, _ptr(regs), len(regions), _ptr(col_ptr), _ptr(col_reg), T,
                                    _ptr(outs[8]), _ptr(outs[16]), _ptr(outs[32]), _ptr(outs[64]), _stream())
            _lib.check(rc, "pww_mask_build")
        else:
            for r in ratios:
                rc = lib.pww_mask_build_rgb(_ptr(rgb), H, W, _ptr(regs), len(regions), _ptr(col_ptr), _ptr(col_reg),
                                            T, r, _ptr(outs[r]), _stream())
                _lib.check(rc, "pww_mask_build_rgb")
    return outs


def mask_build_f32(masks, cols, ratios=(8, 16, 32, 64)):
    _require_gpu(masks)
    masks = masks.to(torch.float32).contiguous()
    R, H, W = masks.shape
    T = len(cols)
    dev = masks.device
    rows = _level_rows(H, W, ratios)
    col_ptr, col_reg = _csr(cols, dev)
    outs = {}
    lib = _lib.load()
    with torch.cuda.device(dev):
        for r in ratios:
            outs[r] = torch.empty((rows[r], T), dtype=torch.float32, device=dev)
        rest = list(ratios)
        if all(r in outs for r in (8, 16, 32, 64)):
            rc = lib.pww_mask_build_f32_levels(_ptr(masks), H, W, R, _ptr(col_ptr), _ptr(col_reg), T, _ptr(outs[8]), _ptr(outs[16]),
                                               _ptr(outs[32]), _ptr(outs[64]), _stream())
            _lib.check(rc, "pww_mask_build_f32_levels")
            rest = [r for r in ratios if r not in (8, 16, 32, 64)]
        for r in rest:
            rc = lib.pww_mask_build_f32(_ptr(masks), H, W, R, _ptr(col_ptr), _ptr(col_reg), T, r, _ptr(outs[r]), _stream())
            _lib.check(rc, "pww_mask_build_f32")
    return outs


def resize_tokens(w_orig, n_tokens):
    import math
    _require_gpu(w_orig)
    if w_orig.dim() != 3 or w_orig.dtype != torch.float32:
        raise PwwHipError("resize_tokens needs an fp32 [H, W, T] map")
    w_orig = w_orig.contiguous()
    H, W, T = w_orig.shape
    ratio = math.sqrt(H * W / n_tokens)
    oh, ow = int(math.floor(H * (1 / ratio))), int(math.floor(W * (1 / ratio)))
    out = torch.empty((n_tokens, T), dtype=torch.float32, device=w_orig.device)
    with torch.cuda.device(w_orig.device):
        _lib.check(_lib.load().pww_resize_tokens(_ptr(w_orig), H, W, T, oh, ow, int(n_tokens), _ptr(out), _stream()), "pww_resize_tokens")
    return out


def gaussian_kernel1d(sigma, ksize=39):
    half = (ksize - 1) * 0.5
    x = torch.linspace(-half, half, steps=ksize, dtype=torch.float32)
    pdf = torch.exp(-0.5 * (x / sigma).pow(2))
    return pdf / pdf.sum()


def gauss_blur(mask, sigma, ksize=39):
    _require_gpu(mask)
    if mask.dim() != 2:
        raise PwwHipError("gauss_blur needs an [H, W] mask")
    mask = mask.to(torch.float32).contiguous()
    H, W = mask.shape
    k = gaussian_kernel1d(float(sigma), ksize).to(mask.device)
    tmp = torch.empty((H, W), dtype=torch.float64, device=mask.device)
    out = torch.empty_like(mask)
    with torch.cuda.device(mask.device):
        _lib.check(_lib.load().pww_gauss_blur(_ptr(mask), _ptr(out), H, W, _ptr(k), int(ksize), _ptr(tmp), _stream()), "pww_gauss_blur")
    return out


def inpaint_prep(rgb, mask, lat_h, lat_w):
    _require_gpu(rgb, mask)
    if rgb.dtype != torch.uint8 or mask.dtype != torch.uint8 or rgb.dim() != 3 or rgb.shape[2] != 3 or tuple(mask.shape) != tuple(rgb.shape[:2]):
        raise PwwHipError("inpaint_prep needs uint8 rgb [H, W, 3] and uint8 mask [H, W]")
    rgb, mask = rgb.contiguous(), mask.contiguous()
    H, W = mask.shape
    dev = rgb.device
    m = torch.empty((1, 1, H, W), dtype=torch.float32, device=dev)
    masked = torch.empty((1, 3, H, W), dtype=torch.float32, device=dev)
    ml = torch.empty((1, 1, lat_h, lat_w), dtype=torch.float32, device=dev)
    with torch.cuda.device(dev):
        _lib.check(_lib.load().pww_inpaint_prep(_ptr(rgb), _ptr(mask), H, W, int(lat_h), int(lat_w), _ptr(m), _ptr(masked), _ptr(ml), _stream()),
                   "pww_inpaint_prep")
    return m, masked, ml


def store_f32(dst, values):
    _require_gpu(dst)
    n = len(values)
    if dst.dtype != torch.float32 or not dst.is_contiguous() or dst.numel() < n:
        raise PwwHipError("store_f32 needs a contiguous float32 device tensor with room for %d values" % n)
    arr = (ctypes.c_float * n)(*[float(v) for v in values])
    with torch.cuda.device(dst.device):
        _lib.check(_lib.load().pww_store_f32(_ptr(dst), arr, n, _stream()), "pww_store_f32")


def cfg_combine(cond, uncond, guidance_scale):
    _require_gpu(cond, uncond)
    if cond.dtype != uncond.dtype or cond.dtype not in _DT or cond.shape != uncond.shape:
        raise PwwHipError("cfg_combine needs two same-shape float16/bfloat16 tensors")
    cond, uncond = cond.contiguous(), uncond.contiguous()
    out = torch.empty(cond.shape, dtype=torch.float32, device=cond.device)
    with torch.cuda.device(cond.device):
        _lib.check(_lib.load().pww_cfg_combine(_ptr(cond), _ptr(uncond), float(guidance_scale), _ptr(out),
                                               cond.numel(), _DT[cond.dtype], _stream()), "pww_cfg_combine")
    return out


def region_masks(rgb, colors, feather=0.0):
    _require_gpu(rgb)
    if rgb.dtype != torch.uint8 or rgb.dim() != 3 or rgb.shape[2] != 3:
        raise PwwHipError("region_masks needs a uint8 colour map [H, W, 3]")
    rgb = rgb.contiguous()
    H, W = int(rgb.shape[0]), int(rgb.shape[1])
    K = len(colors)
    flat = [int(v) for c in colors for v in c]
    if len(flat) != 3 * K or any(not 0 <= v <= 255 for v in flat):
        raise PwwHipError("region_masks needs (r, g, b) colours of 8-bit values")
    host = (ctypes.c_uint8 * max(len(flat), 1))(*flat)
    out = torch.empty((K, H // 8, W // 8), dtype=torch.float32, device=rgb.device)
    lib = _lib.load_regions()
    with torch.cuda.device(rgb.device):
        _lib.check(lib.pww_regions_masks(_ptr(rgb), H, W, host, K, float(feather), _ptr(out), _stream()), "pww_regions_masks", lib)
    return out


def region_combine(eps, masks, weights, scales, guidance_scale):
    _require_gpu(eps, masks, weights, scales)
    if eps.dtype not in _DT or eps.dim() != 4 or masks.dim() != 4:
        raise PwwHipError("region_combine needs a float16 / bfloat16 [(K + 2) n, C, h, w] tensor and fp32 masks [n, K, h, w]")
    n, K = int(masks.shape[0]), int(masks.shape[1])
    if (eps.shape[0] != (K + 2) * n or tuple(eps.shape[-2:]) != tuple(masks.shape[-2:]) or tuple(weights.shape) != (n, K) or tuple(scales.shape) != (n, K)
            or any(t.dtype != torch.float32 for t in (masks, weights, scales))):
        raise PwwHipError("region_combine: eps %s does not go with masks %s, weights %s and scales %s (fp32)"
                          % (tuple(eps.shape), tuple(masks.shape), tuple(weights.shape), tuple(scales.shape)))
    eps, masks, weights, scales = eps.contiguous(), masks.contiguous(), weights.contiguous(), scales.contiguous()
    C, h, w = (int(v) for v in eps.shape[1:])
    out = torch.empty((n, C, h, w), dtype=torch.float32, device=eps.device)
    lib = _lib.load_regions()
    with torch.cuda.device(eps.device):
        _lib.check(lib.pww_regions_combine(_ptr(eps), _ptr(masks), _ptr(weights), _ptr(scales), float(guidance_scale), _ptr(out), n, K, C, h * w,
                                           _DT[eps.dtype], _stream()), "pww_regions_combine", lib)
    return out


def canvas_windows(L, win, stride):
    L, win, stride = int(L), int(win), int(stride)
    if win < 1 or L < win or not 1 <= stride <= win:
        raise ValueError("canvas_windows: length %d, window %d, stride %d (1 <= stride <= window <= length)" % (L, win, stride))
    return tuple(range(0, L - win, stride)) + (L - win,)


def _canvas_origins(ys, xs):
    ys, xs = [int(v) for v in ys], [int(v) for v in xs]
    if not ys or not xs:
        raise PwwHipError("canvas: the window origins ys and xs must not be empty")
    return ys, xs, (ctypes.c_int32 * len(ys))(*ys), (ctypes.c_int32 * len(xs))(*xs)


def canvas_gather(canvas, ys, xs, h, w, denom, copies, dtype):
    _require_gpu(canvas)
    if canvas.dim() == 4 and canvas.shape[0] == 1:
        canvas = canvas[0]
    if canvas.dtype != torch.float32 or canvas.dim() != 3:
        raise PwwHipError("canvas_gather needs a float32 canvas [C, Hc, Wc] (or [1, C, Hc, Wc])")
    if dtype not in _DT:
        raise PwwHipError("canvas_gather: the output type must be float16 or bfloat16 (got %s)" % dtype)
    ys, xs, ys_c, xs_c = _canvas_origins(ys, xs)
    canvas = canvas.contiguous()
    C, Hc, Wc = (int(v) for v in canvas.shape)
    out = torch.empty((int(copies) * len(ys) * len(xs), C, int(h), int(w)), dtype=dtype, device=canvas.device)
    lib = _lib.load_canvas()
    with torch.cuda.device(canvas.device):
        _lib.check(lib.pww_canvas_gather(_ptr(canvas), _ptr(out), ys_c, len(ys), xs_c, len(xs), C, Hc, Wc, int(h), int(w), float(denom), int(copies),
                                         _DT[dtype], _stream()), "pww_canvas_gather", lib)
    return out


def canvas_combine(eps, ys, xs, canvas_hw, guidance_scale, ramp=0, masks=None, weights=None, scales=None):
    _require_gpu(eps, masks, weights, scales)
    ys, xs, ys_c, xs_c = _canvas_origins(ys, xs)
    n_w = len(ys) * len(xs)
    if eps.dtype not in _DT or eps.dim() != 4:
        raise PwwHipError("canvas_combine needs a float16 / bfloat16 [(K + 2) n_w, C, h, w] tensor")
    K = 0
    if masks is not None or weights is not None or scales is not None:
        if masks is None or weights is None or scales is None or masks.dim() != 4:
            raise PwwHipError("canvas_combine: region prompts need masks fp32 [n_w, K, h, w] with weights and scales fp32 [n_w, K]")
        K = int(masks.shape[1])
        if (int(masks.shape[0]) != n_w or tuple(eps.shape[-2:]) != tuple(masks.shape[-2:]) or tuple(weights.shape) != (n_w, K) or tuple(scales.shape) != (n_w, K)
                or any(t.dtype != torch.float32 for t in (masks, weights, scales))):
            raise PwwHipError("canvas_combine: eps %s of %d windows does not go with masks %s, weights %s and scales %s (fp32)"
                              % (tuple(eps.shape), n_w, tuple(masks.shape), tuple(weights.shape), tuple(scales.shape)))
        masks, weights, scales = masks.contiguous(), weights.contiguous(), scales.contiguous()
    if eps.shape[0] != (K + 2) * n_w:
        raise PwwHipError("canvas_combine: eps has %d rows for %d windows and %d regions ((K + 2) n_w = %d)" % (eps.shape[0], n_w, K, (K + 2) * n_w))
    eps = eps.contiguous()
    C, h, w = (int(v) for v in eps.shape[1:])
    Hc, Wc = (int(v) for v in canvas_hw)
    out = torch.empty((1, C, Hc, Wc), dtype=torch.float32, device=eps.device)
    lib = _lib.load_canvas()
    with torch.cuda.device(eps.device):
        _lib.check(lib.pww_canvas_combine(_ptr(eps), _ptr(masks), _ptr(weights), _ptr(scales), float(guidance_scale), _ptr(out), ys_c, len(ys), xs_c,
                                          len(xs), K, C, Hc, Wc, h, w, int(ramp), _DT[eps.dtype], _stream()), "pww_canvas_combine", lib)
    return out


def group_norm(x, num_groups, weight=None, bias=None, eps=1e-5, add=None, act=None, workspace=None, out=None, pre_bias=None):
    _require_gpu(x)
    if x.dim() != 4 or x.dtype not in _DT:
        raise PwwHipError("group_norm needs a 4-d float16/bfloat16 tensor (got %s %s)" % (tuple(x.shape), x.dtype))
    B, C, H, W = x.shape
    if x.is_contiguous():
        layout = _lib.LAYOUT_NCHW
    elif x.is_contiguous(memory_format=torch.channels_last):
        layout = _lib.LAYOUT_NHWC
    else:
        x = x.contiguous()
        layout = _lib.LAYOUT_NCHW
    if out is None:
        out = torch.empty_like(x)
    elif out.shape != x.shape or out.dtype != x.dtype or out.stride() != x.stride():
        raise PwwHipError("group_norm: `out` must have x's shape, dtype and strides")
    for name, t, shape in (("weight", weight, (C,)), ("bias", bias, (C,)), ("add", add, (B, C)), ("pre_bias", pre_bias, (C,))):
        if t is not None and (t.dtype != x.dtype or tuple(t.shape) != shape or t.device != x.device):
            raise PwwHipError("group_norm: `%s` must be %s %s on %s (got %s %s)" % (name, x.dtype, shape, x.device, t.dtype, tuple(t.shape)))
    weight = weight.contiguous() if weight is not None else None
    bias = bias.contiguous() if bias is not None else None
    pre_bias = pre_bias.contiguous() if pre_bias is not None else None
    add_stride = 0
    if add is not None:
        if add.stride(1) != 1 or add.stride(0) % 8 != 0 or add.data_ptr() % 16 != 0:
            add = add.contiguous()
        add_stride = add.stride(0) if B > 1 else C
    if act not in (None, "silu"):
        raise PwwHipError("group_norm: act must be None or 'silu'")
    d = _lib.GnDesc(_DT[x.dtype], layout, B, C, H * W, int(num_groups), float(eps), _lib.ACT_SILU if act == "silu" else _lib.ACT_NONE, add_stride, 0)
    lib = _lib.load()
    need = lib.pww_group_norm_workspace_bytes(ctypes.byref(d))
    if need == 0:
        raise PwwHipError("group_norm: unsupported shape B %d C %d HW %d groups %d (C and H*W multiples of 8, C %% groups == 0, "
                          "groups <= 32, C <= 4096 in channels_last)" % (B, C, H * W, num_groups))
    ws = workspace if workspace is not None else torch.empty(int(need), dtype=torch.uint8, device=x.device)
    with torch.cuda.device(x.device):
        _lib.check(lib.pww_group_norm_fwd(_ptr(x), _ptr(pre_bias), _ptr(add), _ptr(weight), _ptr(bias), _ptr(out), ctypes.byref(d), _ptr(ws), ws.numel(),
                                          _stream()), "pww_group_norm_fwd")
    return out


def _rows(t, name):
    if t.dtype not in _DT or t.dim() < 2:
        raise PwwHipError("%s: a float16/bfloat16 tensor of at least two dims is needed (got %s %s)" % (name, t.dtype, tuple(t.shape)))
    if t.stride(-1) != 1 or t.stride(-2) % 8 != 0 or t.data_ptr() % 16 != 0:
        return None
    C = t.shape[-1]
    rows = t.numel() // C
    stride = t.stride(-2)
    exp = stride
    for d in range(t.dim() - 2, -1, -1):
        if t.shape[d] != 1 and t.stride(d) != exp:
            return None
        exp *= t.shape[d]
    return rows, C, stride


def add_layer_norm(x, weight, bias, eps, a=None, post_bias=None):
    _require_gpu(x)
    rx = _rows(x, "add_layer_norm")
    if rx is None:
        x = x.contiguous()
        rx = _rows(x, "add_layer_norm")
    if rx is None:
        raise PwwHipError("add_layer_norm: the last dim must be a multiple of 8 (got %d)" % x.shape[-1])
    rows, C, xs = rx
    ra = None
    if a is not None:
        if a.shape != x.shape or a.dtype != x.dtype:
            raise PwwHipError("add_layer_norm: `a` must have x's shape and dtype")
        ra = _rows(a, "add_layer_norm")
        if ra is None:
            a = a.contiguous()
            ra = _rows(a, "add_layer_norm")
    for name, t in (("weight", weight), ("bias", bias), ("post_bias", post_bias)):
        if t is not None and (t.dtype != x.dtype or tuple(t.shape) != (C,) or not t.is_contiguous()):
            raise PwwHipError("add_layer_norm: `%s` must be a contiguous %s [%d]" % (name, x.dtype, C))
    if post_bias is not None and a is None:
        raise PwwHipError("add_layer_norm: post_bias needs the add form (a)")
    y = torch.empty(x.shape, dtype=x.dtype, device=x.device)
    s = torch.empty(x.shape, dtype=x.dtype, device=x.device) if a is not None else None
    d = _lib.LnDesc(_DT[x.dtype], C, rows, ra[2] if ra else 0, xs, C, C, float(eps), 0)
    with torch.cuda.device(x.device):
        if post_bias is not None:
            _lib.check(_lib.load().pww_add_layer_norm_bias(_ptr(a), _ptr(x), _ptr(weight), _ptr(bias), _ptr(post_bias), _ptr(s), _ptr(y), ctypes.byref(d),
                                                           _stream()), "pww_add_layer_norm_bias")
        else:
            _lib.check(_lib.load().pww_add_layer_norm(_ptr(a), _ptr(x), _ptr(weight), _ptr(bias), _ptr(s), _ptr(y), ctypes.byref(d), _stream()),
                       "pww_add_layer_norm")
    return (s, y) if a is not None else y


def geglu(h):
    _require_gpu(h)
    r = _rows(h, "geglu")
    if r is None:
        h = h.contiguous()
        r = _rows(h, "geglu")
    if r is None:
        raise PwwHipError("geglu: the last dim must be 2 * D with D a multiple of 8 (got %d)" % h.shape[-1])
    rows, C2, hs = r
    if C2 % 16 != 0:
        raise PwwHipError("geglu: the last dim must be 2 * D with D a multiple of 8 (got %d)" % C2)
    D = C2 // 2
    y = torch.empty(h.shape[:-1] + (D,), dtype=h.dtype, device=h.device)
    with torch.cuda.device(h.device):
        _lib.check(_lib.load().pww_geglu(_ptr(h), _ptr(y), rows, D, hs, D, _DT[h.dtype], _stream()), "pww_geglu")
    return y


def bias_residual(residual, value, bias):
    _require_gpu(residual, value, bias)
    if residual.shape != value.shape or residual.dtype != value.dtype or residual.dtype not in _DT or residual.dim() != 4 or bias.dtype != residual.dtype:
        raise PwwHipError("bias_residual: two same-shape 4-d float16/bfloat16 tensors and a bias of that type are needed")
    B, C, H, W = residual.shape
    if tuple(bias.shape) != (C,):
        raise PwwHipError("bias_residual: bias must have shape (%d,), got %s" % (C, tuple(bias.shape)))
    nhwc = value.is_contiguous(memory_format=torch.channels_last) and not value.is_contiguous()
    fmt = torch.channels_last if nhwc else torch.contiguous_format
    value, residual = value.contiguous(memory_format=fmt), residual.contiguous(memory_format=fmt)
    layout = _lib.LAYOUT_NHWC if nhwc else _lib.LAYOUT_NCHW
    y = torch.empty_like(value)
    with torch.cuda.device(value.device):
        _lib.check(_lib.load().pww_bias_residual(_ptr(residual), _ptr(value), _ptr(bias.contiguous()), _ptr(y), B, C, H * W, layout, _DT[value.dtype], _stream()),
                   "pww_bias_residual")
    return y


def _khwc_weight(weight):
    if weight.is_contiguous(memory_format=torch.channels_last):
        return weight
    key = (weight.data_ptr(), weight._version, weight.dtype, weight.device)
    hit = weight.__dict__.get("_pww_khwc")
    if hit is not None and hit[0] == key:
        return hit[1]
    packed = weight.detach().permute(0, 2, 3, 1).contiguous()
    weight.__dict__["_pww_khwc"] = (key, packed)
    return packed


def conv3x3_takes(x, weight, stride=1, upsample=False):
    if not (torch.is_tensor(x) and x.is_cuda and x.dim() == 4 and x.dtype in _DT and torch.is_tensor(weight) and weight.dtype == x.dtype and weight.dim() == 4):
        return False
    B, C, H, W = x.shape
    Cout = weight.shape[0]
    return (tuple(weight.shape[1:]) == (C, 3, 3) and C % 64 == 0 and Cout % 64 == 0 and stride in (1, 2) and not (upsample and stride != 1)
            and x.is_contiguous(memory_format=torch.channels_last) and x.data_ptr() % 16 == 0
            and B * H * W * C < 2 ** 31 // 4)


def conv3x3(x, weight, bias=None, residual=None, stride=1, upsample=False, tile_n=0, splitk=0):
    _require_gpu(x, weight, bias, residual)
    if not conv3x3_takes(x, weight, stride, upsample):
        raise PwwHipError("conv3x3: needs a channels_last float16/bfloat16 x with Cin, Cout multiples of 64 and a 3 x 3 weight of its dtype")
    B, C, H, W = x.shape
    Cout = weight.shape[0]
    Hv, Wv = H << int(bool(upsample)), W << int(bool(upsample))
    Ho, Wo = (Hv - 1) // stride + 1, (Wv - 1) // stride + 1
    w = _khwc_weight(weight)
    if bias is not None and (bias.dtype != x.dtype or tuple(bias.shape) != (Cout,)):
        raise PwwHipError("conv3x3: bias must be a %s [%d]" % (x.dtype, Cout))
    if bias is not None:
        bias = bias.contiguous()
    if residual is not None:
        if tuple(residual.shape) != (B, Cout, Ho, Wo) or residual.dtype != x.dtype:
            raise PwwHipError("conv3x3: residual must be a %s %s" % (x.dtype, (B, Cout, Ho, Wo)))
        residual = residual.contiguous(memory_format=torch.channels_last)
    d = _lib.ConvDesc(ctypes.sizeof(_lib.ConvDesc), _DT[x.dtype], B, H, W, C, Cout, int(stride), int(bool(upsample)), int(tile_n), int(splitk), 0)
    lib = _lib.load()
    y = torch.empty((B, Cout, Ho, Wo), dtype=x.dtype, device=x.device, memory_format=torch.channels_last)
    nbytes = int(lib.pww_conv3x3_workspace_bytes(ctypes.byref(d)))
    ws = torch.empty(nbytes // 4, dtype=torch.float32, device=x.device) if nbytes else None
    with torch.cuda.device(x.device):
        _lib.check(lib.pww_conv3x3_fwd(_ptr(x), _ptr(w), _ptr(bias), _ptr(residual), _ptr(y), ctypes.byref(d), _ptr(ws), nbytes, _stream()), "pww_conv3x3_fwd")
    return y


def conv3x3_shortcut_takes(h, conv2_weight, x, shortcut_weight):
    if not (conv3x3_takes(h, conv2_weight) and torch.is_tensor(x) and x.is_cuda and x.device == h.device and x.dim() == 4 and x.dtype == h.dtype
            and torch.is_tensor(shortcut_weight) and shortcut_weight.dtype == h.dtype and shortcut_weight.device == h.device):
        return False
    w2 = _linear_weight(shortcut_weight)
    B, C2, H, W = x.shape
    return (w2 is not None and tuple(w2.shape) == (conv2_weight.shape[0], C2) and C2 % 64 == 0 and (B, H, W) == (h.shape[0], h.shape[2], h.shape[3])
            and x.is_contiguous(memory_format=torch.channels_last) and x.data_ptr() % 16 == 0 and B * H * W * C2 < 2 ** 31 // 4)


def conv3x3_shortcut(h, conv2_weight, conv2_bias, x, shortcut_weight, shortcut_bias, tile_n=0, splitk=0):
    _require_gpu(h, conv2_weight, conv2_bias, x, shortcut_weight, shortcut_bias)
    if not conv3x3_shortcut_takes(h, conv2_weight, x, shortcut_weight):
        raise PwwHipError("conv3x3_shortcut: needs channels_last float16/bfloat16 h and x of one dtype, batch and size, channel counts multiples of 64, "
                          "a 3 x 3 weight and a dense 1 x 1 weight of that dtype")
    B, C, H, W = h.shape
    Cout, C2 = conv2_weight.shape[0], x.shape[1]
    w = _khwc_weight(conv2_weight)
    w2 = _linear_weight(shortcut_weight)
    biases = []
    for name, b in (("conv2_bias", conv2_bias), ("shortcut_bias", shortcut_bias)):
        if not torch.is_tensor(b) or b.dtype != h.dtype or tuple(b.shape) != (Cout,):
            raise PwwHipError("conv3x3_shortcut: %s must be a %s [%d]" % (name, h.dtype, Cout))
        biases.append(b.contiguous() if b.data_ptr() % 8 == 0 else b.clone(memory_format=torch.contiguous_format))
    lib = _lib.load_convtail()
    if lib is None:
        raise PwwHipError("conv3x3_shortcut: libpww_hip_convtail.so is not built %s" % _lib._HINT)
    d = _lib.ConvTailDesc(ctypes.sizeof(_lib.ConvTailDesc), _DT[h.dtype], B, H, W, C, C2, Cout, int(tile_n), int(splitk))
    y = torch.empty((B, Cout, H, W), dtype=h.dtype, device=h.device, memory_format=torch.channels_last)
    nbytes = int(lib.pww_convtail_workspace_bytes(ctypes.byref(d)))
    ws = torch.empty(nbytes // 4, dtype=torch.float32, device=h.device) if nbytes else None
    with torch.cuda.device(h.device):
        _lib.check(lib.pww_convtail_fwd(_ptr(h), _ptr(w), _ptr(x), _ptr(w2), _ptr(biases[0]), _ptr(biases[1]), _ptr(y), ctypes.byref(d), _ptr(ws), nbytes,
                                        _stream()), "pww_convtail_fwd", lib)
    return y


def _linear_weight(weight):
    if not torch.is_tensor(weight) or weight.dim() not in (2, 4) or (weight.dim() == 4 and tuple(weight.shape[2:]) != (1, 1)):
        return None
    w = weight.detach().reshape(weight.shape[0], weight.shape[1]) if weight.dim() == 4 else weight.detach()
    return w if w.is_contiguous() and w.data_ptr() == weight.data_ptr() and w.data_ptr() % 16 == 0 else None


def linear_takes(x, weight, geglu=False, bias=None, residual=None, out=None):
    if not (torch.is_tensor(x) and x.is_cuda and x.dtype in _DT and x.dim() >= 2 and torch.is_tensor(weight) and weight.dtype == x.dtype):
        return False
    w = _linear_weight(weight)
    if w is None or x.shape[-1] != w.shape[1] or x.numel() == 0 or _rows(x, "linear") is None:
        return False
    N, K = w.shape
    rows, _, xs = _rows(x, "linear")
    if not (K % 64 == 0 and N % (128 if geglu else 64) == 0 and rows * xs < 2 ** 31 and rows * N < 2 ** 31 and N * K < 2 ** 31):
        return False
    if bias is not None and not (torch.is_tensor(bias) and bias.is_cuda and bias.dtype == x.dtype and tuple(bias.shape) == (N,) and bias.is_contiguous()
                                 and bias.data_ptr() % 8 == 0):
        return False
    shape = tuple(x.shape[:-1]) + (N // 2 if geglu else N,)
    for t in (residual, out):
        if t is not None and not (torch.is_tensor(t) and t.is_cuda and t.dtype == x.dtype and tuple(t.shape) == shape and _rows(t, "linear") is not None):
            return False
    return True


def linear(x, weight, bias=None, residual=None, geglu=False, tile_n=0, splitk=0, out=None):
    _require_gpu(x, weight, bias, residual, out)
    if not linear_takes(x, weight, geglu):
        raise PwwHipError("linear: needs a float16/bfloat16 [..., K] x with one row pitch and a dense [N, K] weight of its dtype, K and N multiples of 64%s"
                          % (" (geglu: N / 2 a multiple of 64)" if geglu else ""))
    w = _linear_weight(weight)
    N, K = w.shape
    M, _, xs = _rows(x, "linear")
    nout = N // 2 if geglu else N
    if (geglu or residual is not None) and bias is None:
        raise PwwHipError("linear: the residual and GEGLU epilogues need the bias")
    if geglu and residual is not None:
        raise PwwHipError("linear: geglu and residual exclude each other")
    if bias is not None:
        if bias.dtype != x.dtype or tuple(bias.shape) != (N,):
            raise PwwHipError("linear: bias must be a %s [%d]" % (x.dtype, N))
        bias = bias.contiguous() if bias.data_ptr() % 8 == 0 else bias.clone(memory_format=torch.contiguous_format)
    shape = tuple(x.shape[:-1]) + (nout,)
    rs = 0
    if residual is not None:
        if tuple(residual.shape) != shape or residual.dtype != x.dtype:
            raise PwwHipError("linear: residual must be a %s %s" % (x.dtype, shape))
        r = _rows(residual, "linear")
        if r is None:
            residual = residual.contiguous()
            r = _rows(residual, "linear")
        rs = r[2]
    if out is None:
        out = torch.empty(shape, dtype=x.dtype, device=x.device)
    elif tuple(out.shape) != shape or out.dtype != x.dtype or _rows(out, "linear") is None:
        raise PwwHipError("linear: out must be a %s %s whose rows have one pitch" % (x.dtype, shape))
    ys = _rows(out, "linear")[2]
    epi = _lib.LINEAR_BIAS_GEGLU if geglu else _lib.LINEAR_BIAS_RESIDUAL if residual is not None else _lib.LINEAR_BIAS if bias is not None else _lib.LINEAR_NONE
    d = _lib.LinearDesc(ctypes.sizeof(_lib.LinearDesc), _DT[x.dtype], M, N, K, epi, xs, ys, rs, int(tile_n), int(splitk))
    lib = _lib.load_linear()
    nbytes = int(lib.pww_linear_workspace_bytes(ctypes.byref(d)))
    ws = torch.empty(nbytes // 4, dtype=torch.float32, device=x.device) if nbytes else None
    with torch.cuda.device(x.device):
        _lib.check(lib.pww_linear_fwd(_ptr(x), _ptr(w), _ptr(bias), _ptr(residual), _ptr(out), ctypes.byref(d), _ptr(ws), nbytes, _stream()), "pww_linear_fwd", lib)
    return out


def lora_update_torch(y, x, A, B, row_adapter, row_scale, n_seg):
    R, ns = y.shape[0], y.shape[-1] // n_seg
    ra, rs = row_adapter[:R].reshape(R, 1, 1), row_scale[:R].reshape(R, 1, 1)
    wide = torch.promote_types(y.dtype, torch.float32)
    for i in range(A.shape[0]):
        on = (ra == i) & (rs != 0)
        for g in range(n_seg):
            u = torch.matmul(torch.matmul(x, A[i, g].t()), B[i, g].t())
            seg = y[..., g * ns:(g + 1) * ns]
            seg.copy_(torch.where(on, (seg.to(wide) + rs.to(wide) * u.to(wide)).to(y.dtype), seg))
    return y


def lora_takes(y, x, A, B, n_seg):
    if not (torch.is_tensor(y) and y.is_cuda and y.dtype in _DT and y.dim() == 3 and x.dim() == 3 and x.dtype == y.dtype == A.dtype == B.dtype
            and x.is_cuda and A.is_cuda and B.is_cuda and A.is_contiguous() and B.is_contiguous() and A.dim() == 4 and B.dim() == 4):
        return False
    (R, T, N), K, (n, seg, rank, _) = y.shape, x.shape[-1], A.shape
    if not (tuple(x.shape[:2]) == (R, T) and seg == n_seg and 1 <= n_seg <= _lib.LORA_MAX_SEGMENTS and 1 <= n <= _lib.LORA_MAX_ADAPTERS and A.shape[3] == K
            and N % n_seg == 0 and tuple(B.shape) == (n, n_seg, N // n_seg, rank) and rank in (32, 64, 96, 128) and K % 32 == 0 and (N // n_seg) % 16 == 0
            and 1 <= R <= 65535 and T >= 1):
        return False
    for t, w in ((x, K), (y, N)):
        rs, ts = (T * t.stride(1) if R == 1 else t.stride(0)), t.stride(1)
        if t.stride(2) != 1 or ts < w or rs < T * ts or rs % 8 or ts % 8 or t.data_ptr() % 16 or R * rs >= 2 ** 31:
            return False
    return A.data_ptr() % 16 == 0 and B.data_ptr() % 16 == 0 and A.numel() < 2 ** 31 and B.numel() < 2 ** 31


def lora_update(y, x, layer_stack, state, n_seg):
    from . import lora as _lora
    A, B = layer_stack
    if x.dtype != y.dtype:
        x = x.to(y.dtype)
    if A.dtype != y.dtype:
        A, B = A.to(y.dtype), B.to(y.dtype)
    if x.dim() == 3 and (x.stride(2) != 1 or x.stride(1) % 8 or (x.shape[0] > 1 and (x.stride(0) % 8 or x.stride(0) < x.shape[1] * x.stride(1))) or x.data_ptr() % 16):
        x = x.contiguous()
    state._ensure_rows()
    if y.shape[0] > state.row_adapter.numel():
        raise PwwHipError("lora_update: %d rows, the assignment holds %d" % (y.shape[0], state.row_adapter.numel()))
    if not lora_takes(y, x, A, B, n_seg):
        _lora._stats["declined"] += 1
        return lora_update_torch(y, x, A, B, state.row_adapter, state.row_scale, n_seg)
    (R, T, N), K = y.shape, x.shape[-1]
    d = _lib.LoraDesc(ctypes.sizeof(_lib.LoraDesc), _DT[y.dtype], R, T, K, N, n_seg, A.shape[2], A.shape[0], 0,
                      T * x.stride(1) if R == 1 else x.stride(0), x.stride(1), T * y.stride(1) if R == 1 else y.stride(0), y.stride(1))
    lib = _lib.load_lora()
    with torch.cuda.device(y.device):
        _lib.check(lib.pww_lora_fwd(_ptr(x), _ptr(A), _ptr(B), _ptr(state.row_adapter), _ptr(state.row_scale), _ptr(y), ctypes.byref(d), _stream()),
                   "pww_lora_fwd", lib)
    _lora._stats["kernel"] += 1
    return y
```

Before: 5.227.

## Eliminate torch.cat in UNet up blocks via concat-aware GroupNorm and conv tail

Adds a side library whose GroupNorm reads two channels_last tensors as if they were concatenated. It also adds a conv2 + 1x1 shortcut kernel that treats x1 and x2 as separate K-slabs. Up-block forwards are patched to pass the skip pair through the resnet instead of materialising torch.cat, which removes the concat copy and its memory traffic. The cost is new kernels that duplicate existing GN and conv-tail logic, falling back to torch.cat when shapes or the library are unsupported.

```diff
diff --git a/include/pww_hip_concat.h b/include/pww_hip_concat.h
--- /dev/null
+++ b/include/pww_hip_concat.h
@@ -0,0 +1,43 @@
+#ifndef PWW_HIP_CONCAT_H
+#define PWW_HIP_CONCAT_H
+
+#include "pww_hip.h"
+
+#ifdef __cplusplus
+extern "C" {
+#endif
+
+#define PWW_CONCAT_VERSION 100
+
+int pww_concat_version(void);
+const char *pww_concat_last_error(void);
+
+typedef struct pww_concat_gn_desc {
+    uint32_t size;
+    int32_t dtype;
+    int32_t B, C1, C2, HW, G;
+    float eps;
+    int32_t act;
+    int32_t _pad;
+} pww_concat_gn_desc_t;
+size_t pww_concat_group_norm_workspace_bytes(const pww_concat_gn_desc_t *desc);
+int pww_concat_group_norm_fwd(const void *x1, const void *x2, const void *gamma, const void *beta, void *y, const pww_concat_gn_desc_t *desc,
+                              void *workspace, size_t workspace_bytes, void *stream);
+
+typedef struct pww_concat_tail_desc {
+    uint32_t size;
+    int32_t dtype;
+    int32_t B, H, W;
+    int32_t Cin, C1, C2, Cout;
+    int32_t tile_n, splitk;
+    int32_t _pad;
+} pww_concat_tail_desc_t;
+size_t pww_concat_convtail_workspace_bytes(const pww_concat_tail_desc_t *desc);
+int pww_concat_convtail_fwd(const void *x, const void *w, const void *x1, const void *x2, const void *wsc, const void *bias, const void *bias2, void *y,
+                            const pww_concat_tail_desc_t *desc, void *workspace, size_t workspace_bytes, void *stream);
+
+#ifdef __cplusplus
+}
+#endif
+
+#endif
diff --git a/paint-with-words-sd_amd/build.py b/paint-with-words-sd_amd/build.py
--- a/paint-with-words-sd_amd/build.py
+++ b/paint-with-words-sd_amd/build.py
@@ -27,6 +27,7 @@
 }
 SIDE_LIBS_EXTRA = {
     "canvas": ("pww_canvas.hip", [], "canvases larger than the UNet's window: the windows' gather and the combine of their noise predictions"),
+    "concat": ("pww_concat.hip", [], "the up blocks without torch.cat: GroupNorm and conv2 + shortcut over the two halves of the concatenation"),
 }
 ALL_SIDE_LIBS = {**SIDE_LIBS, **SIDE_LIBS_CONV, **SIDE_LIBS_EXTRA}
 SOURCES = sorted({u[0] for u in UNITS + EXPERIMENT_UNITS})
@@ -37,6 +38,7 @@
 LONG_UNITS, SCOPE_UNITS, LINEAR_UNITS, REGIONS_UNITS, LORA_UNITS = (SIDE_UNITS[n] for n in ("long", "scope", "linear", "regions", "lora"))
 LIB_CONVTAIL, CONVTAIL_UNITS = SIDE_PATHS["convtail"], SIDE_UNITS["convtail"]
 LIB_CANVAS, CANVAS_UNITS = SIDE_PATHS["canvas"], SIDE_UNITS["canvas"]
+LIB_CONCAT, CONCAT_UNITS = SIDE_PATHS["concat"], SIDE_UNITS["concat"]
 SIDE_PUBLIC_HEADERS = {"canvas": ["pww_hip_regions.h"]}
 HIPCC = os.environ.get("HIPCC", "/opt/rocm/bin/hipcc")
 FLAGS = ["--offload-arch=gfx950", "-O3", "-std=c++17", "-fPIC", "-Wall",
@@ -112,6 +114,7 @@
 def build_lora(force=False, verbose=False): return build_side("lora", force, verbose)
 def build_convtail(force=False, verbose=False): return build_side("convtail", force, verbose)
 def build_canvas(force=False, verbose=False): return build_side("canvas", force, verbose)
+def build_concat(force=False, verbose=False): return build_side("concat", force, verbose)
 
 
 def _build_check(exe, lib, libname, defines, force):
diff --git a/paint-with-words-sd_amd/csrc/pww_concat.hip b/paint-with-words-sd_amd/csrc/pww_concat.hip
--- /dev/null
+++ b/paint-with-words-sd_amd/csrc/pww_concat.hip
@@ -0,0 +1,696 @@
+#define PWW_SIDE_LIB "libpww_hip_concat"
+#include "pww_side_host.h"
+#include "../../include/pww_hip_concat.h"
+
+#define PWW_CONCAT_API extern "C" __attribute__((visibility("default")))
+
+namespace pww {
+
+namespace {
+
+constexpr int GN_NT = 256;
+constexpr int GN_UN = 8;
+constexpr int GN_MAX_SLABS = 64;
+constexpr int GN_GROUP_PIECES = 24;
+
+struct CatGnCold {
+    const void *gamma, *beta;
+    void *y;
+    float eps;
+};
+#define CG_KARGS const void *x1_, const void *x2_, double *partial_, int C1_, int C2_, int HW_, int G_, int cg_, int nslab_, int slab_px_, int apply_px_, const CatGnCold cold_
+struct CatGnParams {
+    const void *x1, *x2, *gamma, *beta;
+    void *y;
+    double *partial;
+    int C1, C2, C, HW, G, cg, nslab, slab_px, apply_px;
+    float eps;
+};
+#define CG_UNPACK const CatGnParams p = {x1_, x2_, cold_.gamma, cold_.beta, cold_.y, partial_, C1_, C2_, C1_ + C2_, HW_, G_, cg_, nslab_, slab_px_, apply_px_, cold_.eps};
+#define CG_LARGS(p) p.x1, p.x2, p.partial, p.C1, p.C2, p.HW, p.G, p.cg, p.nslab, p.slab_px, p.apply_px, CatGnCold{p.gamma, p.beta, p.y, p.eps}
+
+typedef double f64x2 __attribute__((ext_vector_type(2)));
+
+template <typename T> __device__ __forceinline__ float round_to(float v) { return (float)(T)v; }
+
+template <typename T> struct GnPivot { static constexpr bool on = false; };
+template <> struct GnPivot<f16> { static constexpr bool on = true; };
+__device__ __forceinline__ void unpivot(double &S, double &Q, double s, double q, double c, double n) {
+    S += s + n * c;
+    Q += q + 2.0 * c * s + n * c * c;
+}
+
+template <typename T> __device__ __forceinline__ float fma_round(float a, float h, float b) { return round_to<T>(fmaf(a, h, b)); }
+template <> __device__ __forceinline__ float fma_round<f16>(float a, float h, float b) {
+    unsigned r;
+    asm("v_fma_mixlo_f16 %0, %1, %2, %3" : "=v"(r) : "v"(a), "v"(h), "v"(b));
+    return (float)__builtin_bit_cast(f16, (unsigned short)(r & 0xffffu));
+}
+
+template <typename T, int ACT> __device__ __forceinline__ float finish(float h, float a, float b) {
+    float y = fma_round<T>(a, h, b);
+    if (ACT == 1) y = y / (1.f + __expf(-y));
+    return y;
+}
+
+__device__ __forceinline__ void mean_rstd(double S, double Q, double n, float eps, float &mean, float &rstd) {
+    const double m = S / n;
+    double var = Q / n - m * m;
+    var = var > 0.0 ? var : 0.0;
+    mean = (float)m;
+    rstd = (float)(1.0 / sqrt(var + (double)eps));
+}
+
+__device__ __forceinline__ void wg_sum(double &S, double &Q, double (*red)[2], int tid) {
+#pragma unroll
+    for (int off = 32; off > 0; off >>= 1) { S += __shfl_down(S, off); Q += __shfl_down(Q, off); }
+    if ((tid & 63) == 0) { red[tid >> 6][0] = S; red[tid >> 6][1] = Q; }
+    __syncthreads();
+    S = 0.0; Q = 0.0;
+#pragma unroll
+    for (int w = 0; w < GN_NT / 64; ++w) { S += red[w][0]; Q += red[w][1]; }
+}
+
+template <typename T>
+__device__ __forceinline__ const T *cat_source(const CatGnParams &p, int b, int c0, int &pitch) {
+    const bool second = c0 >= p.C1;
+    pitch = second ? p.C2 : p.C1;
+    const T *base = reinterpret_cast<const T *>(second ? p.x2 : p.x1);
+    return base + (long)b * p.HW * pitch + (second ? c0 - p.C1 : c0);
+}
+
+template <typename T, int NT>
+__global__ void __launch_bounds__(NT) cat_gn_moments(CG_KARGS) {
+    CG_UNPACK
+    extern __shared__ __attribute__((aligned(16))) char smem[];
+    typedef typename Vec<T>::v8 V8;
+    const int tid = threadIdx.x, b = blockIdx.y, slab = blockIdx.x;
+    const int CH = p.C >> 3, PL = NT / CH;
+    const int pl = tid / CH, ch = tid - pl * CH;
+    float *ls = reinterpret_cast<float *>(smem);
+    float *lq = ls + PL * p.C;
+    double *lk = reinterpret_cast<double *>(lq + PL * p.C);
+
+    if (pl < PL) {
+        float s[8], q[8];
+#pragma unroll
+        for (int j = 0; j < 8; ++j) s[j] = q[j] = 0.f;
+        int pitch;
+        const T *x = cat_source<T>(p, b, ch * 8, pitch);
+        float c = 0.f;
+        const int p0 = slab * p.slab_px, p1 = min(p0 + p.slab_px, p.HW);
+#pragma unroll 1
+        for (int px = p0 + pl; px < p1; px += GN_UN * PL) {
+            V8 r[GN_UN];
+#pragma unroll
+            for (int u = 0; u < GN_UN; ++u) {
+                const int pu = px + u * PL;
+                r[u] = *reinterpret_cast<const V8 *>(x + (long)(pu < p1 ? pu : px) * pitch);
+            }
+            if constexpr (GnPivot<T>::on) {
+                if (px == p0 + pl) c = (float)r[0][0];
+            }
+#pragma unroll
+            for (int u = 0; u < GN_UN; ++u) {
+                const bool ok = px + u * PL < p1;
+#pragma unroll
+                for (int j = 0; j < 8; ++j) {
+                    float h = (float)r[u][j];
+                    if constexpr (GnPivot<T>::on) h -= c;
+                    h = ok ? h : 0.f;
+                    s[j] += h;
+                    q[j] = fmaf(h, h, q[j]);
+                }
+            }
+        }
+#pragma unroll
+        for (int j = 0; j < 8; ++j) { ls[pl * p.C + ch * 8 + j] = s[j]; lq[pl * p.C + ch * 8 + j] = q[j]; }
+        if constexpr (GnPivot<T>::on) reinterpret_cast<float *>(lk + (NT / p.G) * p.G * 2)[tid] = c;
+    }
+    __syncthreads();
+    const int K = NT / p.G, g = tid % p.G, k = tid / p.G;
+    if (k < K) {
+        double S = 0.0, Q = 0.0;
+        const int n = PL * p.cg;
+        for (int e = k; e < n; e += K) {
+            const int r = e / p.cg, c = g * p.cg + (e - r * p.cg);
+            if constexpr (GnPivot<T>::on) {
+                const float *lc = reinterpret_cast<const float *>(lk + K * p.G * 2);
+                const int p0 = slab * p.slab_px, p1 = min(p0 + p.slab_px, p.HW);
+                const int cnt = p0 + r < p1 ? (p1 - p0 - r + PL - 1) / PL : 0;
+                unpivot(S, Q, (double)ls[r * p.C + c], (double)lq[r * p.C + c], (double)lc[r * CH + (c >> 3)], (double)cnt);
+            } else {
+                S += (double)ls[r * p.C + c]; Q += (double)lq[r * p.C + c];
+            }
+        }
+        lk[(k * p.G + g) * 2] = S; lk[(k * p.G + g) * 2 + 1] = Q;
+    }
+    __syncthreads();
+    if (tid < p.G) {
+        double S = 0.0, Q = 0.0;
+        for (int r = 0; r < K; ++r) { S += lk[(r * p.G + tid) * 2]; Q += lk[(r * p.G + tid) * 2 + 1]; }
+        f64x2 v; v[0] = S; v[1] = Q;
+        reinterpret_cast<f64x2 *>(p.partial)[((long)b * p.nslab + slab) * p.G + tid] = v;
+    }
+}
+
+template <typename T, int ACT, int NT>
+__global__ void __launch_bounds__(NT) cat_gn_apply(CG_KARGS) {
+    CG_UNPACK
+    extern __shared__ __attribute__((aligned(16))) char smem[];
+    typedef typename Vec<T>::v8 V8;
+    constexpr int NPART = 8;
+    const int tid = threadIdx.x, b = blockIdx.y;
+    const int CH = p.C >> 3, PL = NT / CH;
+    const int pl = tid / CH, ch = tid - pl * CH;
+    const bool active = pl < PL;
+    double *lk = reinterpret_cast<double *>(smem);
+    const int K = NT / p.G, g = tid % p.G, k = tid / p.G;
+    float *stat = reinterpret_cast<float *>(lk + K * p.G * 2);
+
+    f64x2 part[NPART];
+#pragma unroll
+    for (int i = 0; i < NPART; ++i) {
+        const int sl = k + i * K;
+        part[i] = reinterpret_cast<const f64x2 *>(p.partial)[((long)b * p.nslab + (k < K && sl < p.nslab ? sl : 0)) * p.G + g];
+    }
+    const int c0 = ch * 8;
+    V8 gv = zero8<V8>(), bv = zero8<V8>();
+    int pitch;
+    const T *x = cat_source<T>(p, b, c0, pitch);
+    T *y = reinterpret_cast<T *>(p.y) + (long)b * p.HW * p.C + c0;
+    const int p0 = blockIdx.x * p.apply_px, p1 = min(p0 + p.apply_px, p.HW);
+    V8 r[GN_UN];
+    if (active) {
+        if (p.gamma) gv = *reinterpret_cast<const V8 *>(reinterpret_cast<const T *>(p.gamma) + c0);
+        if (p.beta) bv = *reinterpret_cast<const V8 *>(reinterpret_cast<const T *>(p.beta) + c0);
+#pragma unroll
+        for (int u = 0; u < GN_UN; ++u) {
+            const int pu = p0 + pl + u * PL;
+            r[u] = *reinterpret_cast<const V8 *>(x + (long)(pu < p1 ? pu : p0) * pitch);
+        }
+    }
+    if (k < K) {
+        double S = 0.0, Q = 0.0;
+#pragma unroll
+        for (int i = 0; i < NPART; ++i)
+            if (k + i * K < p.nslab) { S += part[i][0]; Q += part[i][1]; }
+        lk[(k * p.G + g) * 2] = S; lk[(k * p.G + g) * 2 + 1] = Q;
+    }
+    __syncthreads();
+    if (tid < p.G) {
+        double S = 0.0, Q = 0.0;
+        for (int rr = 0; rr < K; ++rr) { S += lk[(rr * p.G + tid) * 2]; Q += lk[(rr * p.G + tid) * 2 + 1]; }
+        float mean, rstd;
+        mean_rstd(S, Q, (double)p.cg * (double)p.HW, p.eps, mean, rstd);
+        stat[tid * 2] = mean; stat[tid * 2 + 1] = rstd;
+    }
+    __syncthreads();
+    if (!active) return;
+    float a[8], bb[8];
+#pragma unroll
+    for (int j = 0; j < 8; ++j) {
+        const int gg = (c0 + j) / p.cg;
+        a[j] = stat[gg * 2 + 1] * (p.gamma ? (float)gv[j] : 1.f);
+        bb[j] = (p.beta ? (float)bv[j] : 0.f) - a[j] * stat[gg * 2];
+    }
+    for (int px = p0 + pl; px < p1; px += GN_UN * PL) {
+        if (px != p0 + pl) {
+#pragma unroll
+            for (int u = 0; u < GN_UN; ++u) {
+                const int pu = px + u * PL;
+                r[u] = *reinterpret_cast<const V8 *>(x + (long)(pu < p1 ? pu : px) * pitch);
+            }
+        }
+#pragma unroll
+        for (int u = 0; u < GN_UN; ++u) {
+            V8 o;
+#pragma unroll
+            for (int j = 0; j < 8; ++j) o[j] = (T)finish<T, ACT>((float)r[u][j], a[j], bb[j]);
+            if (px + u * PL < p1) *reinterpret_cast<V8 *>(y + (long)(px + u * PL) * p.C) = o;
+        }
+    }
+}
+
+template <typename T, int ACT>
+__global__ void __launch_bounds__(GN_NT) cat_gn_group(CG_KARGS) {
+    CG_UNPACK
+    typedef T TV __attribute__((ext_vector_type(4)));
+    __shared__ double red[GN_NT / 64][2];
+    const int tid = threadIdx.x, g = blockIdx.x, b = blockIdx.y;
+    const int ppp = p.cg >> 2, PLs = GN_NT / ppp;
+    const int pl = tid / ppp, sub = tid - pl * ppp;
+    const bool active = pl < PLs;
+    const int pc = pl < p.HW ? pl : 0;
+    const int c0 = g * p.cg + sub * 4;
+    int pitch;
+    const T *x = cat_source<T>(p, b, c0, pitch);
+    T *y = reinterpret_cast<T *>(p.y) + (long)b * p.HW * p.C + c0;
+    TV raw[GN_GROUP_PIECES];
+    const TV z = {(T)0.f, (T)0.f, (T)0.f, (T)0.f};
+    TV gv = z, bv = z;
+    if (active) {
+#pragma unroll
+        for (int j = 0; j < GN_GROUP_PIECES; ++j) {
+            const int px = pl + j * PLs;
+            raw[j] = *reinterpret_cast<const TV *>(x + (long)(px < p.HW ? px : pc) * pitch);
+        }
+        if (p.gamma) gv = *reinterpret_cast<const TV *>(reinterpret_cast<const T *>(p.gamma) + c0);
+        if (p.beta) bv = *reinterpret_cast<const TV *>(reinterpret_cast<const T *>(p.beta) + c0);
+    }
+    float v[GN_GROUP_PIECES][4];
+    float s = 0.f, q = 0.f, c = 0.f;
+    int cnt = 0;
+    if (active) {
+#pragma unroll
+        for (int j = 0; j < GN_GROUP_PIECES; ++j) {
+            const bool ok = pl + j * PLs < p.HW;
+#pragma unroll
+            for (int e = 0; e < 4; ++e) {
+                float h = (float)raw[j][e];
+                h = ok ? h : 0.f;
+                v[j][e] = h;
+                if constexpr (GnPivot<T>::on) {
+                    if (j == 0 && e == 0) c = h;
+                    h = ok ? h - c : 0.f;
+                }
+                s += h;
+                q = fmaf(h, h, q);
+            }
+            if constexpr (GnPivot<T>::on) cnt += ok ? 4 : 0;
+        }
+    }
+    double S = (double)s, Q = (double)q;
+    if constexpr (GnPivot<T>::on) { S = 0.0; Q = 0.0; unpivot(S, Q, (double)s, (double)q, (double)c, (double)cnt); }
+    wg_sum(S, Q, red, tid);
+    float mean, rstd;
+    mean_rstd(S, Q, (double)p.cg * (double)p.HW, p.eps, mean, rstd);
+    if (!active) return;
+    float a[4], bb[4];
+#pragma unroll
+    for (int e = 0; e < 4; ++e) {
+        a[e] = rstd * (p.gamma ? (float)gv[e] : 1.f);
+        bb[e] = (p.beta ? (float)bv[e] : 0.f) - a[e] * mean;
+    }
+#pragma unroll
+    for (int j = 0; j < GN_GROUP_PIECES; ++j) {
+        const int px = pl + j * PLs;
+        if (px < p.HW) {
+            TV o;
+#pragma unroll
+            for (int e = 0; e < 4; ++e) o[e] = (T)finish<T, ACT>(v[j][e], a[e], bb[e]);
+            *reinterpret_cast<TV *>(y + (long)px * p.C) = o;
+        }
+    }
+}
+
+struct CatGnPlan { int nslab, slab_px, apply_px, nt; bool group; size_t partial_bytes, lds_m, lds_a; };
+
+bool desc_ok(const void *d, uint32_t size, size_t want, const char *what) {
+    if (d && size >= want) return true;
+    set_error("%s: descriptor missing or older than this library (size %u)", what, d ? size : 0u);
+    return false;
+}
+
+bool cat_gn_plan(const pww_concat_gn_desc_t *d, CatGnPlan &pl) {
+    const long C = (long)d->C1 + d->C2;
+    const bool ok = d->B >= 1 && d->B <= 65535 && d->C1 >= 8 && d->C2 >= 8 && d->C1 % 8 == 0 && d->C2 % 8 == 0 && C <= 4096 && d->HW >= 8 && d->HW % 8 == 0
+                    && d->G >= 1 && d->G <= 32 && C % d->G == 0 && (d->dtype == PWW_DTYPE_F16 || d->dtype == PWW_DTYPE_BF16)
+                    && (d->act == PWW_ACT_NONE || d->act == PWW_ACT_SILU) && (long)d->B * d->HW * C < (1L << 40);
+    if (!ok) {
+        set_error("concat_group_norm: unsupported (dtype %d B %d C1 %d C2 %d HW %d G %d act %d): C1, C2 and HW multiples of 8, (C1 + C2) %% G == 0, "
+                  "G <= 32, C1 + C2 <= 4096", d->dtype, d->B, d->C1, d->C2, d->HW, d->G, d->act);
+        return false;
+    }
+    pl = CatGnPlan();
+    const int Ct = (int)C, cg = Ct / d->G, CH = Ct / 8;
+    pl.nt = CH <= 256 ? 256 : 512;
+    const int PL = pl.nt / CH;
+    if (cg % 4 == 0 && cg / 4 <= GN_NT) {
+        const int PLs = GN_NT / (cg / 4);
+        pl.group = (d->HW + PLs - 1) / PLs <= GN_GROUP_PIECES;
+    }
+    int px = (d->HW + GN_MAX_SLABS - 1) / GN_MAX_SLABS;
+    if (px < GN_UN * PL) px = GN_UN * PL;
+    if (px > d->HW) px = d->HW;
+    pl.slab_px = px;
+    pl.nslab = (d->HW + px - 1) / px;
+    int want = (512 + d->B - 1) / d->B;
+    int apx = (d->HW + want - 1) / want;
+    if (apx < GN_UN * PL) apx = GN_UN * PL;
+    if (apx > d->HW) apx = d->HW;
+    pl.apply_px = apx;
+    pl.partial_bytes = (size_t)d->B * pl.nslab * d->G * 2 * sizeof(double);
+    const size_t lk = (size_t)(pl.nt / d->G) * d->G * 2 * sizeof(double);
+    pl.lds_m = (size_t)2 * PL * Ct * sizeof(float) + lk + (d->dtype == PWW_DTYPE_F16 ? (size_t)pl.nt * sizeof(float) : 0);
+    pl.lds_a = lk + (size_t)d->G * 2 * sizeof(float);
+    return true;
+}
+
+template <typename T>
+int cat_gn_launch(const CatGnParams &p, const pww_concat_gn_desc_t *d, const CatGnPlan &pl, hipStream_t stream) {
+    const bool silu = d->act == PWW_ACT_SILU;
+    if (pl.group) {
+        const dim3 grid(d->G, d->B);
+        if (silu) hipLaunchKernelGGL((cat_gn_group<T, 1>), grid, dim3(GN_NT), 0, stream, CG_LARGS(p));
+        else hipLaunchKernelGGL((cat_gn_group<T, 0>), grid, dim3(GN_NT), 0, stream, CG_LARGS(p));
+        return check_hip(hipGetLastError(), "concat_group_norm launch");
+    }
+    const dim3 gm(pl.nslab, d->B), ga((d->HW + pl.apply_px - 1) / pl.apply_px, d->B);
+    if (pl.nt == 256) {
+        hipLaunchKernelGGL((cat_gn_moments<T, 256>), gm, dim3(256), pl.lds_m, stream, CG_LARGS(p));
+        if (silu) hipLaunchKernelGGL((cat_gn_apply<T, 1, 256>), ga, dim3(256), pl.lds_a, stream, CG_LARGS(p));
+        else hipLaunchKernelGGL((cat_gn_apply<T, 0, 256>), ga, dim3(256), pl.lds_a, stream, CG_LARGS(p));
+    } else {
+        hipLaunchKernelGGL((cat_gn_moments<T, 512>), gm, dim3(512), pl.lds_m, stream, CG_LARGS(p));
+        if (silu) hipLaunchKernelGGL((cat_gn_apply<T, 1, 512>), ga, dim3(512), pl.lds_a, stream, CG_LARGS(p));
+        else hipLaunchKernelGGL((cat_gn_apply<T, 0, 512>), ga, dim3(512), pl.lds_a, stream, CG_LARGS(p));
+    }
+    return check_hip(hipGetLastError(), "concat_group_norm launch");
+}
+
+constexpr int CT_BM = 128, CT_THREADS = 256;
+constexpr int CT_PF = 2;
+
+__device__ __forceinline__ f32x4 mfma16(f16x8 a, f16x8 b, f32x4 c) { return __builtin_amdgcn_mfma_f32_16x16x32_f16(a, b, c, 0, 0, 0); }
+__device__ __forceinline__ f32x4 mfma16(bf16x8 a, bf16x8 b, f32x4 c) { return __builtin_amdgcn_mfma_f32_16x16x32_bf16(a, b, c, 0, 0, 0); }
+
+struct CatTailCold {
+    const void *x1, *x2, *wsc, *bias, *bias2;
+    int nsplit, nmain, ntail;
+};
+
+__device__ __forceinline__ int xcd_remap(int orig, int nwg) {
+    const int xcd = orig & 7, q = nwg >> 3, r = nwg & 7;
+    return (xcd < r ? xcd * (q + 1) : r * (q + 1) + (xcd - r) * q) + (orig >> 3);
+}
+
+template <typename T>
+__device__ __forceinline__ void epilogue4(const f32x4 &a, const CatTailCold &cold, T *y, long off, int n) {
+    typedef typename Vec<T>::v4 V4;
+    const V4 b = *reinterpret_cast<const V4 *>(reinterpret_cast<const T *>(cold.bias) + n);
+    const V4 b2 = *reinterpret_cast<const V4 *>(reinterpret_cast<const T *>(cold.bias2) + n);
+    V4 o;
+#pragma unroll
+    for (int j = 0; j < 4; ++j) o[j] = (T)(a[j] + (float)b[j] + (float)b2[j]);
+    *reinterpret_cast<V4 *>(y + off) = o;
+}
+
+template <typename T, int BN>
+__global__ void __launch_bounds__(CT_THREADS, 2) cat_tail_kernel(const T *__restrict__ x, const T *__restrict__ w, void *__restrict__ out, int M, int N,
+                                                                 int Cin, int C1, int C2, int H, int W, const CatTailCold cold) {
+    typedef typename Vec<T>::v8 V8;
+    constexpr int BM = CT_BM, PF = CT_PF, XL = BM * 8 / CT_THREADS, WL = BN * 8 / CT_THREADS, RM = 4, RN = BN / 32;
+    constexpr int XBYTES = BM * 128, STAGE = (BM + BN) * 128;
+    __shared__ __attribute__((aligned(16))) char lds[2 * STAGE];
+
+    const int tid = threadIdx.x, lane = tid & 63, wave = tid >> 6, wm = wave >> 1, wn = wave & 1;
+    const int ntm = (M + BM - 1) / BM;
+    const int bid = xcd_remap(blockIdx.x, gridDim.x);
+    const bool split = cold.nsplit > 1;
+    const int tile = bid / cold.nsplit, ks = bid - tile * cold.nsplit;
+    const int tm = tile % ntm, tn = tile / ntm;
+    const int nmain = cold.nmain, nslab = nmain + cold.ntail;
+    const int s_begin = (int)((long)ks * nslab / cold.nsplit), s_end = (int)((long)(ks + 1) * nslab / cold.nsplit);
+    const int K9 = 9 * Cin, HW = H * W, Ct = C1 + C2;
+    const T *__restrict__ xa = reinterpret_cast<const T *>(cold.x1);
+    const T *__restrict__ xb2 = reinterpret_cast<const T *>(cold.x2);
+    const T *__restrict__ w2 = reinterpret_cast<const T *>(cold.wsc);
+
+    const int c = tid & 7;
+    int pix[XL], y0[XL], x0[XL];
+#pragma unroll
+    for (int i = 0; i < XL; ++i) {
+        int m = tm * BM + (tid >> 3) + 32 * i;
+        m = m < M ? m : M - 1;
+        const int b = m / HW, rem = m - b * HW, oy = rem / W, ox = rem - oy * W;
+        pix[i] = b * HW;
+        y0[i] = oy - 1;
+        x0[i] = ox - 1;
+    }
+    const unsigned wrow = (unsigned)(tn * BN + (tid >> 3));
+    const unsigned woff_main = wrow * (unsigned)K9 + c * 8, woff_tail = wrow * (unsigned)Ct + c * 8;
+    const int swz = ((c ^ ((tid >> 3) & 7)) << 4);
+
+    u32x4 xr[PF][XL], wr[PF][WL];
+    unsigned xok[PF];
+    const bool tail0 = s_begin >= nmain;
+    int tap = tail0 ? 9 : s_begin / (Cin >> 6);
+    int ci0 = tail0 ? (s_begin - nmain) << 6 : (s_begin - tap * (Cin >> 6)) << 6;
+    int kmain = s_begin * 64;
+    const bool second0 = tail0 && ci0 >= C1;
+    const T *xs = second0 ? xb2 - C1 : xa;
+    int ps = second0 ? C2 : C1;
+    auto load = [&](int p) {
+        const bool tail = tap >= 9;
+        const int ky = tail ? 1 : tap / 3, kx = tail ? 1 : tap - (tap / 3) * 3;
+        const T *xb = tail ? xs : x;
+        const T *wb = tail ? w2 : w;
+        const int pitch = tail ? ps : Cin;
+        const unsigned wpitch = (unsigned)(tail ? Ct : K9);
+        const unsigned wo = (tail ? woff_tail : woff_main) + (unsigned)(tail ? ci0 : kmain);
+        xok[p] = 0;
+#pragma unroll
+        for (int i = 0; i < XL; ++i) {
+            const int iy = y0[i] + ky, ix = x0[i] + kx;
+            const bool ok = (unsigned)iy < (unsigned)H && (unsigned)ix < (unsigned)W;
+            xr[p][i] = *reinterpret_cast<const u32x4 *>(xb + (unsigned)((pix[i] + (ok ? iy : 0) * W + (ok ? ix : 0)) * pitch + ci0 + c * 8));
+            xok[p] |= (unsigned)ok << i;
+        }
+#pragma unroll
+        for (int j = 0; j < WL; ++j) wr[p][j] = *reinterpret_cast<const u32x4 *>(wb + (wo + (unsigned)(32 * j) * wpitch));
+        kmain += 64;
+        ci0 += 64;
+        const bool wrap = ci0 == Cin && !tail;
+        ci0 = wrap ? 0 : ci0;
+        tap += wrap ? 1 : 0;
+        const bool cross = ci0 == C1 && tail;
+        xs = cross ? xb2 - C1 : xs;
+        ps = cross ? C2 : ps;
+    };
+    auto store = [&](int p, int buf) {
+        char *base = lds + buf * STAGE;
+#pragma unroll
+        for (int i = 0; i < XL; ++i) {
+            const u32x4 z = {0u, 0u, 0u, 0u};
+            *reinterpret_cast<u32x4 *>(base + ((tid >> 3) + 32 * i) * 128 + swz) = (xok[p] >> i) & 1u ? xr[p][i] : z;
+        }
+#pragma unroll
+        for (int j = 0; j < WL; ++j) *reinterpret_cast<u32x4 *>(base + XBYTES + ((tid >> 3) + 32 * j) * 128 + swz) = wr[p][j];
+    };
+
+    f32x4 acc[RN][RM];
+#pragma unroll
+    for (int r = 0; r < RN; ++r)
+#pragma unroll
+        for (int i = 0; i < RM; ++i) acc[r][i] = f32x4{0.f, 0.f, 0.f, 0.f};
+
+    const int fr = lane & 15, fq = lane >> 4;
+    auto compute = [&](int buf) {
+        const char *bx = lds + buf * STAGE, *bw = bx + XBYTES;
+#pragma unroll
+        for (int kk = 0; kk < 2; ++kk) {
+            V8 xf[RM], wf[RN];
+#pragma unroll
+            for (int q = 0; q < RM; ++q) {
+                const int row = wm * 64 + q * 16 + fr;
+                xf[q] = *reinterpret_cast<const V8 *>(bx + row * 128 + (((kk * 4 + fq) ^ (row & 7)) << 4));
+            }
+#pragma unroll
+            for (int r = 0; r < RN; ++r) {
+                const int row = wn * (BN / 2) + r * 16 + fr;
+                wf[r] = *reinterpret_cast<const V8 *>(bw + row * 128 + (((kk * 4 + fq) ^ (row & 7)) << 4));
+            }
+#pragma unroll
+            for (int r = 0; r < RN; ++r)
+#pragma unroll
+                for (int q = 0; q < RM; ++q) acc[r][q] = mfma16(wf[r], xf[q], acc[r][q]);
+        }
+    };
+
+    const int n = s_end - s_begin;
+    load(0);
+#pragma unroll
+    for (int p = 1; p < PF; ++p)
+        if (p < n) load(p);
+    store(0, 0);
+    __syncthreads();
+    int i = 0;
+    for (; i + 2 * PF <= n; i += PF) {
+#pragma unroll
+        for (int p = 0; p < PF; ++p) {
+            load(p);
+            compute((i + p) & 1);
+            __builtin_amdgcn_sched_barrier(0);
+            store((p + 1) % PF, (i + p + 1) & 1);
+            __syncthreads();
+        }
+    }
+#pragma unroll
+    for (int t = 0; t < 2 * PF - 1; ++t) {
+        if (i + t < n) {
+            if (i + t + PF < n) load(t % PF);
+            compute((i + t) & 1);
+            if (i + t + 1 < n) store((t + 1) % PF, (i + t + 1) & 1);
+            __syncthreads();
+        }
+    }
+
+#pragma unroll
+    for (int i = 0; i < RM; ++i) {
+        const int m = tm * BM + wm * 64 + i * 16 + fr;
+        if (m >= M) continue;
+#pragma unroll
+        for (int r = 0; r < RN; ++r) {
+            const int n = tn * BN + wn * (BN / 2) + r * 16 + fq * 4;
+            if (split) *reinterpret_cast<f32x4 *>(reinterpret_cast<float *>(out) + ((long)ks * M + m) * N + n) = acc[r][i];
+            else epilogue4<T>(acc[r][i], cold, reinterpret_cast<T *>(out), (long)m * N + n, n);
+        }
+    }
+}
+
+template <typename T>
+__global__ void __launch_bounds__(256) cat_tail_fold_kernel(const float *__restrict__ ws, T *__restrict__ y, long n4, int N, long MN, const CatTailCold cold) {
+    const long q = (long)blockIdx.x * 256 + threadIdx.x;
+    if (q >= n4) return;
+    const long off = q * 4;
+    f32x4 a = *reinterpret_cast<const f32x4 *>(ws + off);
+    for (int s = 1; s < cold.nsplit; ++s) a += *reinterpret_cast<const f32x4 *>(ws + s * MN + off);
+    epilogue4<T>(a, cold, y, off, (int)(off % N));
+}
+
+struct TailTune { int M, N, nmain, ntail, bn, nsplit; };
+constexpr TailTune TAIL_TUNED[] = {
+    {128, 1280, 180, 40, 64, 12},
+    {512, 1280, 180, 40, 128, 12}, {512, 1280, 180, 30, 128, 12}, {512, 1280, 180, 10, 128, 12},
+    {2048, 640, 90, 30, 128, 6}, {2048, 640, 90, 20, 128, 6}, {2048, 640, 90, 15, 128, 6}, {2048, 640, 90, 5, 128, 6},
+    {8192, 320, 45, 15, 64, 4}, {8192, 320, 45, 10, 64, 4},
+};
+
+struct TailPlan {
+    int M, bn, nsplit, nmain, ntail, ntiles;
+};
+
+bool cat_tail_plan(const pww_concat_tail_desc_t *d, TailPlan *p) {
+    if ((d->dtype != PWW_DTYPE_F16 && d->dtype != PWW_DTYPE_BF16) || d->B < 1 || d->H < 1 || d->W < 1 || d->Cin < 64 || d->Cin % 64 != 0 || d->C1 < 64
+        || d->C1 % 64 != 0 || d->C2 < 64 || d->C2 % 64 != 0 || d->Cout < 64 || d->Cout % 64 != 0 || d->Cin > 65536 || d->C1 > 32768 || d->C2 > 32768
+        || d->Cout > 65536) {
+        set_error("concat_convtail: unsupported (dtype %d B %d %dx%d Cin %d C1 %d C2 %d Cout %d): Cin, C1, C2 and Cout multiples of 64", d->dtype, d->B,
+                  d->H, d->W, d->Cin, d->C1, d->C2, d->Cout);
+        return false;
+    }
+    const long M = (long)d->B * d->H * d->W, Ct = (long)d->C1 + d->C2;
+    if (M * d->Cin >= (1L << 31) || M * Ct >= (1L << 31) || M * d->Cout >= (1L << 31) || 9L * d->Cin * d->Cout >= (1L << 31) || Ct * d->Cout >= (1L << 31)) {
+        set_error("concat_convtail: tensor of 2^31 elements or more");
+        return false;
+    }
+    p->M = (int)M;
+    p->nmain = 9 * d->Cin / 64;
+    p->ntail = (int)(Ct / 64);
+    const int nslab = p->nmain + p->ntail;
+    const TailTune *tuned = nullptr;
+    for (const TailTune &t : TAIL_TUNED)
+        if (t.M == p->M && t.N == d->Cout && t.nmain == p->nmain && t.ntail == p->ntail) tuned = &t;
+    p->bn = d->tile_n ? d->tile_n : tuned ? tuned->bn : (d->Cout % 128 == 0 ? 128 : 64);
+    if ((p->bn != 64 && p->bn != 128) || d->Cout % p->bn != 0) { set_error("concat_convtail: tile_n %d does not divide Cout %d", d->tile_n, d->Cout); return false; }
+    p->ntiles = (p->M + CT_BM - 1) / CT_BM * (d->Cout / p->bn);
+    int ns = d->splitk;
+    if (ns <= 0 && tuned && p->bn == tuned->bn) ns = tuned->nsplit;
+    if (ns <= 0) {
+        ns = (480 + p->ntiles / 2) / p->ntiles;
+        if (ns > nslab / 8) ns = nslab / 8;
+        if (ns < 1) ns = 1;
+    }
+    if (ns > nslab || ns > 64) { set_error("concat_convtail: split %d exceeds the %d K-slabs (or 64)", ns, nslab); return false; }
+    p->nsplit = ns;
+    return true;
+}
+
+template <typename T>
+int cat_tail_launch(const TailPlan &p, const pww_concat_tail_desc_t *d, const void *x, const void *w, const CatTailCold &cold, void *y, void *ws,
+                    hipStream_t stream) {
+    const T *xt = static_cast<const T *>(x), *wt = static_cast<const T *>(w);
+    const int N = d->Cout;
+    const dim3 grid(p.ntiles * p.nsplit), block(CT_THREADS);
+    void *out = p.nsplit == 1 ? y : ws;
+    if (p.bn == 128) launch_timed(cat_tail_kernel<T, 128>, grid, block, 0, stream, xt, wt, out, p.M, N, d->Cin, d->C1, d->C2, d->H, d->W, cold);
+    else launch_timed(cat_tail_kernel<T, 64>, grid, block, 0, stream, xt, wt, out, p.M, N, d->Cin, d->C1, d->C2, d->H, d->W, cold);
+    if (p.nsplit == 1) return check_hip(hipGetLastError(), "concat_convtail launch");
+    const long MN = (long)p.M * N, n4 = MN / 4;
+    launch_timed(cat_tail_fold_kernel<T>, dim3((unsigned)((n4 + 255) / 256)), dim3(256), 0, stream, static_cast<const float *>(ws), static_cast<T *>(y), n4,
+                 N, MN, cold);
+    return check_hip(hipGetLastError(), "concat_convtail fold launch");
+}
+
+}
+
+size_t concat_group_norm_workspace_bytes(const pww_concat_gn_desc_t *d) {
+    CatGnPlan pl;
+    if (!desc_ok(d, d ? d->size : 0u, sizeof(pww_concat_gn_desc_t), "concat_group_norm") || !cat_gn_plan(d, pl)) return 0;
+    return pl.group ? 16 : pl.partial_bytes;
+}
+
+int concat_group_norm_fwd(const void *x1, const void *x2, const void *gamma, const void *beta, void *y, const pww_concat_gn_desc_t *d, void *workspace,
+                          size_t workspace_bytes, hipStream_t stream) {
+    if (!desc_ok(d, d ? d->size : 0u, sizeof(pww_concat_gn_desc_t), "concat_group_norm")) return PWW_EINVAL;
+    CatGnPlan pl;
+    if (!cat_gn_plan(d, pl)) return PWW_ENOTSUP;
+    if (!x1 || !x2 || !y || !workspace) { set_error("concat_group_norm: x1, x2, y and workspace are required"); return PWW_EINVAL; }
+    if (!aligned16(x1) || !aligned16(x2) || !aligned16(y) || !aligned16(workspace) || !aligned16(gamma) || !aligned16(beta)) {
+        set_error("concat_group_norm: pointers must be 16-byte aligned");
+        return PWW_EINVAL;
+    }
+    const size_t need = pl.group ? 16 : pl.partial_bytes;
+    if (workspace_bytes < need) { set_error("concat_group_norm: workspace of %zu bytes, need %zu", workspace_bytes, need); return PWW_EINVAL; }
+    if (!arch_ok()) return PWW_ENOTSUP;
+    CatGnParams p;
+    p.x1 = x1; p.x2 = x2; p.gamma = gamma; p.beta = beta; p.y = y;
+    p.partial = static_cast<double *>(workspace);
+    p.C1 = d->C1; p.C2 = d->C2; p.C = d->C1 + d->C2; p.HW = d->HW; p.G = d->G; p.cg = p.C / d->G;
+    p.nslab = pl.nslab; p.slab_px = pl.slab_px; p.apply_px = pl.apply_px;
+    p.eps = d->eps;
+    return d->dtype == PWW_DTYPE_F16 ? cat_gn_launch<f16>(p, d, pl, stream) : cat_gn_launch<bf16>(p, d, pl, stream);
+}
+
+size_t concat_convtail_workspace_bytes(const pww_concat_tail_desc_t *d) {
+    TailPlan p;
+    if (!desc_ok(d, d ? d->size : 0u, sizeof(pww_concat_tail_desc_t), "concat_convtail") || !cat_tail_plan(d, &p)) return 0;
+    return p.nsplit > 1 ? (size_t)p.nsplit * p.M * d->Cout * sizeof(float) : 0;
+}
+
+int concat_convtail_fwd(const void *x, const void *w, const void *x1, const void *x2, const void *wsc, const void *bias, const void *bias2, void *y,
+                        const pww_concat_tail_desc_t *d, void *workspace, size_t workspace_bytes, hipStream_t stream) {
+    if (!desc_ok(d, d ? d->size : 0u, sizeof(pww_concat_tail_desc_t), "concat_convtail")) return PWW_EINVAL;
+    TailPlan p;
+    if (!cat_tail_plan(d, &p)) return PWW_ENOTSUP;
+    if (!x || !w || !x1 || !x2 || !wsc || !bias || !bias2 || !y) { set_error("concat_convtail: x, w, x1, x2, wsc, bias, bias2 and y are required"); return PWW_EINVAL; }
+    if (!aligned16(x) || !aligned16(w) || !aligned16(x1) || !aligned16(x2) || !aligned16(wsc) || !aligned16(y) || (reinterpret_cast<uintptr_t>(bias) & 7)
+        || (reinterpret_cast<uintptr_t>(bias2) & 7)) {
+        set_error("concat_convtail: x, w, x1, x2, wsc, y must be 16-byte aligned, the biases 8-byte aligned");
+        return PWW_EINVAL;
+    }
+    const size_t need = p.nsplit > 1 ? (size_t)p.nsplit * p.M * d->Cout * sizeof(float) : 0;
+    if (need && (!workspace || !aligned16(workspace) || workspace_bytes < need)) {
+        set_error("concat_convtail: split %d needs a 16-byte aligned workspace of %zu bytes (got %zu)", p.nsplit, need, workspace_bytes);
+        return PWW_EINVAL;
+    }
+    if (!arch_ok()) return PWW_ENOTSUP;
+    const CatTailCold cold{x1, x2, wsc, bias, bias2, p.nsplit, p.nmain, p.ntail};
+    if (d->dtype == PWW_DTYPE_F16) return cat_tail_launch<f16>(p, d, x, w, cold, y, workspace, stream);
+    return cat_tail_launch<bf16>(p, d, x, w, cold, y, workspace, stream);
+}
+
+}
+
+PWW_CONCAT_API int pww_concat_version(void) { return PWW_CONCAT_VERSION; }
+PWW_CONCAT_API const char *pww_concat_last_error(void) { return pww::last_error(); }
+PWW_CONCAT_API size_t pww_concat_group_norm_workspace_bytes(const pww_concat_gn_desc_t *desc) { return pww::concat_group_norm_workspace_bytes(desc); }
+PWW_CONCAT_API int pww_concat_group_norm_fwd(const void *x1, const void *x2, const void *gamma, const void *beta, void *y, const pww_concat_gn_desc_t *desc,
+                                             void *workspace, size_t workspace_bytes, void *stream) {
+    return pww::concat_group_norm_fwd(x1, x2, gamma, beta, y, desc, workspace, workspace_bytes, static_cast<hipStream_t>(stream));
+}
+PWW_CONCAT_API size_t pww_concat_convtail_workspace_bytes(const pww_concat_tail_desc_t *desc) { return pww::concat_convtail_workspace_bytes(desc); }
+PWW_CONCAT_API int pww_concat_convtail_fwd(const void *x, const void *w, const void *x1, const void *x2, const void *wsc, const void *bias, const void *bias2,
+                                           void *y, const pww_concat_tail_desc_t *desc, void *workspace, size_t workspace_bytes, void *stream) {
+    return pww::concat_convtail_fwd(x, w, x1, x2, wsc, bias, bias2, y, desc, workspace, workspace_bytes, static_cast<hipStream_t>(stream));
+}
diff --git a/paint-with-words-sd_amd/pww_hip/_lib.py b/paint-with-words-sd_amd/pww_hip/_lib.py
--- a/paint-with-words-sd_amd/pww_hip/_lib.py
+++ b/paint-with-words-sd_amd/pww_hip/_lib.py
@@ -12,6 +12,7 @@
 LORA_LIB_PATH = os.environ.get("PWW_HIP_LORA_LIB", os.path.join(_HERE, "libpww_hip_lora.so"))
 CONVTAIL_LIB_PATH = os.environ.get("PWW_HIP_CONVTAIL_LIB", os.path.join(_HERE, "libpww_hip_convtail.so"))
 CANVAS_LIB_PATH = os.environ.get("PWW_HIP_CANVAS_LIB", os.path.join(_HERE, "libpww_hip_canvas.so"))
+CONCAT_LIB_PATH = os.environ.get("PWW_HIP_CONCAT_LIB", os.path.join(_HERE, "libpww_hip_concat.so"))
 
 PWW_OK, PWW_EINVAL, PWW_ENOTSUP, PWW_EHIP = 0, -22, -95, -5
 MIN_VERSION = 127
@@ -67,6 +68,11 @@
 CANVAS_MAX_WINDOWS, CANVAS_MAX_RAMP, CANVAS_MIN_WINDOW, CANVAS_MAX_WINDOW = 64, 64, 8, 128
 
 
+CONCAT_EXPORTS = ("pww_concat_version", "pww_concat_last_error", "pww_concat_group_norm_workspace_bytes", "pww_concat_group_norm_fwd",
+                  "pww_concat_convtail_workspace_bytes", "pww_concat_convtail_fwd")
+CONCAT_MIN_VERSION = 100
+
+
 class AttnDesc(ctypes.Structure):
     _fields_ = [("dtype", ctypes.c_int32), ("B", ctypes.c_int32), ("H", ctypes.c_int32), ("N", ctypes.c_int32),
                 ("M", ctypes.c_int32), ("D", ctypes.c_int32),
@@ -123,6 +129,17 @@
 class ConvTailDesc(ctypes.Structure):
     _fields_ = [("size", ctypes.c_uint32), ("dtype", ctypes.c_int32), ("B", ctypes.c_int32), ("H", ctypes.c_int32), ("W", ctypes.c_int32),
                 ("Cin", ctypes.c_int32), ("C2", ctypes.c_int32), ("Cout", ctypes.c_int32), ("tile_n", ctypes.c_int32), ("splitk", ctypes.c_int32)]
+
+
+class ConcatGnDesc(ctypes.Structure):
+    _fields_ = [("size", ctypes.c_uint32), ("dtype", ctypes.c_int32), ("B", ctypes.c_int32), ("C1", ctypes.c_int32), ("C2", ctypes.c_int32),
+                ("HW", ctypes.c_int32), ("G", ctypes.c_int32), ("eps", ctypes.c_float), ("act", ctypes.c_int32), ("_pad", ctypes.c_int32)]
+
+
+class ConcatTailDesc(ctypes.Structure):
+    _fields_ = [("size", ctypes.c_uint32), ("dtype", ctypes.c_int32), ("B", ctypes.c_int32), ("H", ctypes.c_int32), ("W", ctypes.c_int32),
+                ("Cin", ctypes.c_int32), ("C1", ctypes.c_int32), ("C2", ctypes.c_int32), ("Cout", ctypes.c_int32), ("tile_n", ctypes.c_int32),
+                ("splitk", ctypes.c_int32), ("_pad", ctypes.c_int32)]
 
 
 class Region(ctypes.Structure):
@@ -297,6 +314,11 @@
     "canvas": dict(path="CANVAS_LIB_PATH", exports=CANVAS_EXPORTS, min_version=CANVAS_MIN_VERSION, missing_ok=False, needs="canvases larger than the window need it", sigs={
         "pww_canvas_gather": ([_vp, _vp, _P(_i32), _i32, _P(_i32), _i32, _i32, _i32, _i32, _i32, _i32, _f32, _i32, _i32, _vp], _int),
         "pww_canvas_combine": ([_vp, _vp, _vp, _vp, _f32, _vp, _P(_i32), _i32, _P(_i32), _i32, _i32, _i32, _i32, _i32, _i32, _i32, _i32, _i32, _vp], _int)}),
+    "concat": dict(path="CONCAT_LIB_PATH", exports=CONCAT_EXPORTS, min_version=CONCAT_MIN_VERSION, missing_ok=True, needs="the up blocks without torch.cat need it", sigs={
+        "pww_concat_group_norm_workspace_bytes": ([_P(ConcatGnDesc)], _sz),
+        "pww_concat_group_norm_fwd": ([_vp, _vp, _vp, _vp, _vp, _P(ConcatGnDesc), _vp, _sz, _vp], _int),
+        "pww_concat_convtail_workspace_bytes": ([_P(ConcatTailDesc)], _sz),
+        "pww_concat_convtail_fwd": ([_vp, _vp, _vp, _vp, _vp, _vp, _vp, _vp, _P(ConcatTailDesc), _vp, _sz, _vp], _int)}),
 }
 _side = {}
 
@@ -372,6 +394,11 @@
     return lib if lib is not None else load_side("canvas")
 
 
+def load_concat():
+    lib = _side.get("concat")
+    return lib if lib is not None else load_side("concat")
+
+
 class experiments:
 
     def __enter__(self):
diff --git a/paint-with-words-sd_amd/pww_hip/blocks.py b/paint-with-words-sd_amd/pww_hip/blocks.py
--- a/paint-with-words-sd_amd/pww_hip/blocks.py
+++ b/paint-with-words-sd_amd/pww_hip/blocks.py
@@ -15,10 +15,11 @@
 LINEAR = os.environ.get("PWW_LINEAR", "1")
 CONV3X3 = os.environ.get("PWW_CONV3X3", "1") != "0"
 CONV_SHORTCUT = os.environ.get("PWW_CONV_SHORTCUT", "1") != "0"
-
-
-_STATS = {k: [0, 0] for k in ("group_norm", "resnet_block", "transformer_block", "geglu", "conv1x1", "conv3x3", "linear", "conv_shortcut")}
-_UNRATED = ("conv1x1", "conv3x3", "linear", "conv_shortcut")
+CONCAT = os.environ.get("PWW_CONCAT", "1") != "0"
+
+
+_STATS = {k: [0, 0] for k in ("group_norm", "resnet_block", "transformer_block", "geglu", "conv1x1", "conv3x3", "linear", "conv_shortcut", "concat")}
+_UNRATED = ("conv1x1", "conv3x3", "linear", "conv_shortcut", "concat")
 _warned = set()
 
 
@@ -146,9 +147,17 @@
         _count("resnet_block", False, input_tensor, ("a call beyond (input_tensor, temb): %d positional, keywords %s" % (len(args), sorted(kwargs))) if not covered else _why_not(input_tensor))
         return self._pww_orig_forward(*args, **kwargs)
     temb = args[1] if len(args) == 2 else kwargs.get("temb")
+    return _resnet_body(self, input_tensor, temb)
+
+
+def _resnet_body(self, input_tensor, temb, pair=None):
     _count("resnet_block", True)
-    fold = FOLD_CONV_BIAS and _plain_conv(self.conv1) and _plain_conv(self.conv2) and self.conv1.bias.dtype == input_tensor.dtype
-    h = fused_group_norm(self.norm1, input_tensor, act="silu")
+    dtype = pair[0].dtype if pair is not None else input_tensor.dtype
+    fold = FOLD_CONV_BIAS and _plain_conv(self.conv1) and _plain_conv(self.conv2) and self.conv1.bias.dtype == dtype
+    if pair is not None:
+        h = ops.group_norm_cat(pair[0], pair[1], self.norm1.num_groups, self.norm1.weight, self.norm1.bias, self.norm1.eps, act="silu")
+    else:
+        h = fused_group_norm(self.norm1, input_tensor, act="silu")
     if fold and _conv3x3_route(self.conv1, h):
         h = ops.conv3x3(h, self.conv1.weight)
     else:
@@ -173,6 +182,14 @@
         h = dropout(h)
     scale = getattr(self, "output_scale_factor", 1.0)
     shortcut = getattr(self, "conv_shortcut", None)
+    if pair is not None:
+        took = shortcut is not None and _conv_shortcut_route(self, shortcut, h, None, fold, scale, pair=pair)
+        _STATS["concat"][0 if took else 1] += 1
+        if took:
+            return ops.conv3x3_shortcut_cat(h, self.conv2.weight, self.conv2.bias, pair[0], pair[1], shortcut.weight, shortcut.bias)
+        input_tensor = torch.cat(pair, dim=1)
+        if shortcut is not None:
+            _STATS["conv_shortcut"][1] -= 1
     if shortcut is not None:
         if _conv_shortcut_route(self, shortcut, h, input_tensor, fold, scale):
             return ops.conv3x3_shortcut(h, self.conv2.weight, self.conv2.bias, input_tensor, shortcut.weight, shortcut.bias)
@@ -202,15 +219,21 @@
     return ok
 
 
-def _conv_shortcut_route(block, shortcut, h, x, fold, scale):
+def _conv_shortcut_route(block, shortcut, h, x, fold, scale, pair=None):
     own = shortcut.__dict__.get("forward")
     ok = (CONV_SHORTCUT and fold and scale == 1.0 and _is_conv1x1(shortcut) and shortcut.bias is not None
           and (own is None or getattr(own, "__func__", None) is _conv1x1_forward) and not shortcut._forward_hooks and not shortcut._forward_pre_hooks
-          and torch.is_tensor(x) and x.dim() == 4 and x.dtype == h.dtype == shortcut.weight.dtype == shortcut.bias.dtype
-          and x.is_contiguous(memory_format=torch.channels_last)
-          and not (torch.is_grad_enabled() and (x.requires_grad or shortcut.weight.requires_grad))
-          and _is_conv3x3(block.conv2) and block.conv2.stride == (1, 1) and ops.conv3x3_shortcut_takes(h, block.conv2.weight, x, shortcut.weight)
-          and ops._lib.load_convtail() is not None)
+          and _is_conv3x3(block.conv2) and block.conv2.stride == (1, 1))
+    if ok and pair is not None:
+        ok = (all(t.dtype == h.dtype == shortcut.weight.dtype == shortcut.bias.dtype for t in pair)
+              and not (torch.is_grad_enabled() and (pair[0].requires_grad or pair[1].requires_grad or shortcut.weight.requires_grad))
+              and ops.conv3x3_shortcut_cat_takes(h, block.conv2.weight, pair[0], pair[1], shortcut.weight))
+    elif ok:
+        ok = (torch.is_tensor(x) and x.dim() == 4 and x.dtype == h.dtype == shortcut.weight.dtype == shortcut.bias.dtype
+              and x.is_contiguous(memory_format=torch.channels_last)
+              and not (torch.is_grad_enabled() and (x.requires_grad or shortcut.weight.requires_grad))
+              and ops.conv3x3_shortcut_takes(h, block.conv2.weight, x, shortcut.weight)
+              and ops._lib.load_convtail() is not None)
     if ok:
         ok = _conv3x3_route(block.conv2, h)
         if not ok:
@@ -342,6 +365,75 @@
     _count("geglu", False, h, _why_not(h))
     a, gate = h.chunk(2, dim=-1)
     return a * F.gelu(gate)
+
+
+_UP_BLOCKS = {
+    "UpBlock": ("x", "skips", "temb", "ctx"),
+    "UpBlock2D": ("hidden_states", "res_hidden_states_tuple", "temb", "upsample_size"),
+    "CrossAttnUpBlock2D": ("hidden_states", "res_hidden_states_tuple", "temb", "encoder_hidden_states", "upsample_size"),
+}
+
+
+def _no_hooks(m):
+    return not m._forward_hooks and not m._forward_pre_hooks and not nn.modules.module._global_forward_hooks and not nn.modules.module._global_forward_pre_hooks
+
+
+def _resnet_cat(res, x1, x2, temb):
+    own = res.__dict__.get("forward")
+    shortcut = getattr(res, "conv_shortcut", None)
+    ok = (CONCAT and CONV_SHORTCUT and FUSED_NORM and getattr(own, "__func__", None) is _resnet_forward and _no_hooks(res)
+          and torch.is_tensor(x1) and torch.is_tensor(x2) and x1.dtype == x2.dtype and not torch.is_autocast_enabled()
+          and not (torch.is_grad_enabled() and (x1.requires_grad or x2.requires_grad))
+          and (temb is None or torch.is_tensor(temb))
+          and shortcut is not None and _is_conv1x1(shortcut) and shortcut.bias is not None and getattr(res, "output_scale_factor", 1.0) == 1.0
+          and x1.dim() == 4 and x2.dim() == 4 and x1.shape[1] % 64 == 0 and x2.shape[1] % 64 == 0
+          and x1.shape[1] + x2.shape[1] == res.norm1.num_channels == shortcut.in_channels
+          and res.norm1.weight is not None and res.norm1.weight.dtype == x1.dtype
+          and not (torch.is_grad_enabled() and res.norm1.weight.requires_grad)
+          and FOLD_CONV_BIAS and _plain_conv(res.conv1) and _plain_conv(res.conv2) and res.conv1.bias.dtype == x1.dtype
+          and _is_conv3x3(res.conv2) and res.conv2.stride == (1, 1) and res.conv2.weight.dtype == x1.dtype
+          and res.conv2.in_channels % 64 == 0 and res.conv2.out_channels % 64 == 0
+          and x1.shape[0] * x1.shape[2] * x1.shape[3] < STOCK_FROM_ROWS
+          and ops.group_norm_cat_takes(x1, x2, res.norm1.num_groups, res.norm1.weight, res.norm1.bias))
+    if ok:
+        return _resnet_body(res, None, temb, pair=(x1, x2))
+    _STATS["concat"][1] += 1
+    return res(torch.cat([x1, x2], dim=1), temb)
+
+
+def _up_block_covered(m):
+    res, att, ups = getattr(m, "resnets", None), getattr(m, "attentions", None), getattr(m, "upsamplers", None)
+    return (m.__class__.__name__ in _UP_BLOCKS and isinstance(res, nn.ModuleList) and len(res) > 0
+            and (att is None or (isinstance(att, nn.ModuleList) and len(att) == len(res))) and (ups is None or isinstance(ups, nn.ModuleList))
+            and (m.__class__.__name__ != "CrossAttnUpBlock2D" or att is not None))
+
+
+def _up_block_forward(self, *args, **kwargs):
+    names = _UP_BLOCKS[self.__class__.__name__]
+    standin = self.__class__.__name__ == "UpBlock"
+    vals = dict(zip(names, args))
+    known = CONCAT and len(args) <= len(names) and all(k in names and k not in vals for k in kwargs) and _no_hooks(self)
+    if known:
+        vals.update(kwargs)
+        skips = vals.get(names[1])
+        known = (names[0] in vals and isinstance(skips, (tuple, list)) and len(skips) >= len(self.resnets) and (not standin or len(vals) == len(names))
+                 and not (self.training and getattr(self, "gradient_checkpointing", False)))
+    if not known:
+        return self._pww_orig_forward(*args, **kwargs)
+    x, temb = vals[names[0]], vals.get("temb")
+    attentions, upsamplers = getattr(self, "attentions", None), getattr(self, "upsamplers", None)
+    for i, res in enumerate(self.resnets):
+        x = _resnet_cat(res, x, skips[-1], temb)
+        skips = skips[:-1]
+        if attentions is not None:
+            x = attentions[i](x, vals["ctx"]) if standin else attentions[i](x, encoder_hidden_states=vals.get("encoder_hidden_states")).sample
+    if upsamplers is not None:
+        if standin:
+            x = upsamplers[0](x)
+        else:
+            for up in upsamplers:
+                x = up(x, vals.get("upsample_size"))
+    return (x, skips) if standin else x
 
 
 def install_blocks(unet):
@@ -374,6 +466,8 @@
             owned.add(id(_upsample_conv(m)))
         elif _is_conv3x3(m) and id(m) not in owned:
             fwd = _conv3x3_forward
+        elif name in _UP_BLOCKS and _up_block_covered(m):
+            fwd = _up_block_forward
         if fwd is not None and "_pww_orig_forward" not in m.__dict__:
             m.__dict__["_pww_orig_forward"] = m.forward
             m.forward = types.MethodType(fwd, m)
diff --git a/paint-with-words-sd_amd/pww_hip/ops.py b/paint-with-words-sd_amd/pww_hip/ops.py
--- a/paint-with-words-sd_amd/pww_hip/ops.py
+++ b/paint-with-words-sd_amd/pww_hip/ops.py
@@ -1046,6 +1046,90 @@
     return y
 
 
+def _cat_pair(x1, x2, grid):
+    if not (torch.is_tensor(x1) and torch.is_tensor(x2) and x1.is_cuda and x1.device == x2.device and x1.dim() == 4 and x2.dim() == 4
+            and x1.dtype in _DT and x2.dtype == x1.dtype):
+        return False
+    (B, C1, H, W), C2 = x1.shape, x2.shape[1]
+    return ((x2.shape[0], x2.shape[2], x2.shape[3]) == (B, H, W) and C1 % grid == 0 and C2 % grid == 0 and C1 > 0 and C2 > 0
+            and x1.is_contiguous(memory_format=torch.channels_last) and x2.is_contiguous(memory_format=torch.channels_last)
+            and x1.data_ptr() % 16 == 0 and x2.data_ptr() % 16 == 0)
+
+
+def _gn_cat_desc(x1, x2, num_groups, eps, act):
+    B, C1, H, W = x1.shape
+    return _lib.ConcatGnDesc(ctypes.sizeof(_lib.ConcatGnDesc), _DT[x1.dtype], B, C1, x2.shape[1], H * W, int(num_groups), float(eps),
+                             _lib.ACT_SILU if act == "silu" else _lib.ACT_NONE, 0)
+
+
+def group_norm_cat_takes(x1, x2, num_groups, weight=None, bias=None):
+    if not _cat_pair(x1, x2, 8):
+        return False
+    C = x1.shape[1] + x2.shape[1]
+    for t in (weight, bias):
+        if t is not None and not (torch.is_tensor(t) and t.dtype == x1.dtype and tuple(t.shape) == (C,) and t.device == x1.device):
+            return False
+    lib = _lib.load_concat()
+    return lib is not None and int(lib.pww_concat_group_norm_workspace_bytes(ctypes.byref(_gn_cat_desc(x1, x2, num_groups, 1e-5, None)))) > 0
+
+
+def group_norm_cat(x1, x2, num_groups, weight=None, bias=None, eps=1e-5, act=None, workspace=None):
+    _require_gpu(x1, x2)
+    if act not in (None, "silu"):
+        raise PwwHipError("group_norm_cat: act must be None or 'silu'")
+    if not group_norm_cat_takes(x1, x2, num_groups, weight, bias):
+        raise PwwHipError("group_norm_cat: needs two channels_last float16/bfloat16 tensors of one dtype, batch and size with channel counts multiples "
+                          "of 8, C1 + C2 a shape group_norm takes, and libpww_hip_concat.so %s" % _lib._HINT)
+    B, C1, H, W = x1.shape
+    weight = weight.contiguous() if weight is not None else None
+    bias = bias.contiguous() if bias is not None else None
+    d = _gn_cat_desc(x1, x2, num_groups, eps, act)
+    lib = _lib.load_concat()
+    need = int(lib.pww_concat_group_norm_workspace_bytes(ctypes.byref(d)))
+    ws = workspace if workspace is not None else torch.empty(need, dtype=torch.uint8, device=x1.device)
+    out = torch.empty((B, C1 + x2.shape[1], H, W), dtype=x1.dtype, device=x1.device, memory_format=torch.channels_last)
+    with torch.cuda.device(x1.device):
+        _lib.check(lib.pww_concat_group_norm_fwd(_ptr(x1), _ptr(x2), _ptr(weight), _ptr(bias), _ptr(out), ctypes.byref(d), _ptr(ws), ws.numel(), _stream()),
+                   "pww_concat_group_norm_fwd", lib)
+    return out
+
+
+def conv3x3_shortcut_cat_takes(h, conv2_weight, x1, x2, shortcut_weight):
+    if not (conv3x3_takes(h, conv2_weight) and _cat_pair(x1, x2, 64) and x1.device == h.device and x1.dtype == h.dtype
+            and torch.is_tensor(shortcut_weight) and shortcut_weight.dtype == h.dtype and shortcut_weight.device == h.device):
+        return False
+    w2 = _linear_weight(shortcut_weight)
+    B, C1, H, W = x1.shape
+    Ct = C1 + x2.shape[1]
+    return (w2 is not None and tuple(w2.shape) == (conv2_weight.shape[0], Ct) and (B, H, W) == (h.shape[0], h.shape[2], h.shape[3])
+            and B * H * W * Ct < 2 ** 31 // 4 and _lib.load_concat() is not None)
+
+
+def conv3x3_shortcut_cat(h, conv2_weight, conv2_bias, x1, x2, shortcut_weight, shortcut_bias, tile_n=0, splitk=0):
+    _require_gpu(h, conv2_weight, conv2_bias, x1, x2, shortcut_weight, shortcut_bias)
+    if not conv3x3_shortcut_cat_takes(h, conv2_weight, x1, x2, shortcut_weight):
+        raise PwwHipError("conv3x3_shortcut_cat: needs channels_last float16/bfloat16 h, x1 and x2 of one dtype, batch and size, channel counts multiples "
+                          "of 64, a 3 x 3 weight and a dense 1 x 1 weight of that dtype over C1 + C2 channels, and libpww_hip_concat.so %s" % _lib._HINT)
+    B, C, H, W = h.shape
+    Cout = conv2_weight.shape[0]
+    w = _khwc_weight(conv2_weight)
+    w2 = _linear_weight(shortcut_weight)
+    biases = []
+    for name, b in (("conv2_bias", conv2_bias), ("shortcut_bias", shortcut_bias)):
+        if not torch.is_tensor(b) or b.dtype != h.dtype or tuple(b.shape) != (Cout,):
+            raise PwwHipError("conv3x3_shortcut_cat: %s must be a %s [%d]" % (name, h.dtype, Cout))
+        biases.append(b.contiguous() if b.data_ptr() % 8 == 0 else b.clone(memory_format=torch.contiguous_format))
+    lib = _lib.load_concat()
+    d = _lib.ConcatTailDesc(ctypes.sizeof(_lib.ConcatTailDesc), _DT[h.dtype], B, H, W, C, x1.shape[1], x2.shape[1], Cout, int(tile_n), int(splitk), 0)
+    y = torch.empty((B, Cout, H, W), dtype=h.dtype, device=h.device, memory_format=torch.channels_last)
+    nbytes = int(lib.pww_concat_convtail_workspace_bytes(ctypes.byref(d)))
+    ws = torch.empty(nbytes // 4, dtype=torch.float32, device=h.device) if nbytes else None
+    with torch.cuda.device(h.device):
+        _lib.check(lib.pww_concat_convtail_fwd(_ptr(h), _ptr(w), _ptr(x1), _ptr(x2), _ptr(w2), _ptr(biases[0]), _ptr(biases[1]), _ptr(y), ctypes.byref(d),
+                                               _ptr(ws), nbytes, _stream()), "pww_concat_convtail_fwd", lib)
+    return y
+
+
 def _linear_weight(weight):
     if not torch.is_tensor(weight) or weight.dim() not in (2, 4) or (weight.dim() == 4 and tuple(weight.shape[2:]) != (1, 1)):
         return None
```

Result: faster. 5.301 (median of 6 runs) (+1.4%).
